# yuan-xy/Audio-Triangulation

Measured on AMD Instinct MI355X. Metric: GCC-PHAT localizations/sec, 3-mic x 1024-sample frames, higher is better.
Workload: dtype f32

## Files before the change

audio-triangulation_amd/csrc/tdoa_capi.cpp:

```cpp

#include "../../include/tdoa.h"
#include "tdoa_devmem.h"
#include "tdoa_internal.h"
#include "tdoa_tables.h"

#include <hip/hip_runtime.h>

#include <cstdlib>

#include <algorithm>
#include <cmath>
#include <cstring>
#include <map>
#include <memory>
#include <mutex>
#include <tuple>
#include <vector>

struct tdoa_ctx {
    tdoa_tables t;
    int device;
    tdoa_devmem window, prior, tuples, tuple_cell, mic, lut;
    tdoa_devmem tw;
    tdoa_devmem p1k_img;
    tdoa_devmem w64_img;
    tdoa_devmem bb;
    tdoa_devmem wc;
    tdoa_devmem fgq;
    tdoa_devmem wscratch;
    tdoa_devmem rscratch, cscratch, tscratch;
    tdoa_devmem pscratch;
    tdoa_devmem spec;
    std::vector<float> bin_w;
    tdoa_devmem d_bin_w;
    tdoa_kparams kp;
};

extern "C" int tdoa_config_default(tdoa_config *cfg)
{
    if (!cfg)
        return tdoa_fail(TDOA_ERR_INVALID, "tdoa_config_default: NULL");
    std::memset(cfg, 0, sizeof *cfg);
    cfg->num_mics = 3;
    cfg->frame_len = 1024;
    cfg->sample_rate_hz = 50000;
    cfg->max_shift = 0;
    cfg->speed_of_sound = 343.0f;
    cfg->engine = TDOA_ENGINE_DIRECT;
    cfg->mic_xy = nullptr;
    cfg->grid_half_w = 50;
    cfg->grid_half_h = 50;
    cfg->grid_scale = 24.0f;
    cfg->height_offset = 1.2f;
    cfg->window_q15 = nullptr;
    cfg->phat_eps = 1e-12f;
    return TDOA_OK;
}

namespace {

int check_device(int device)
{
    int ndev = 0;
    if (hipGetDeviceCount(&ndev) != hipSuccess || ndev <= 0)
        return tdoa_fail(TDOA_ERR_NO_DEVICE, "no HIP device visible (libtdoa has no CPU path)");
    if (device < 0 || device >= ndev)
        return tdoa_fail(TDOA_ERR_INVALID, "device %d out of range (%d visible)", device, ndev);
    hipDeviceProp_t prop;
    HIP_TRY(hipGetDeviceProperties(&prop, device));
    if (std::strncmp(prop.gcnArchName, "gfx950", 6) != 0)
        return tdoa_fail(TDOA_ERR_NO_DEVICE, "device %d is %s; libtdoa is built for gfx950 only",
                         device, prop.gcnArchName);
    return TDOA_OK;
}

template <typename T> size_t vbytes(const std::vector<T> &v) { return v.size() * sizeof(T); }

int upload_tables(tdoa_ctx *c)
{
    const tdoa_tables &t = c->t;
    std::vector<int16_t> w16(t.N);
    for (int i = 0; i < t.N; i++)
        w16[i] = (int16_t)t.win[i];
    if (c->window.alloc(vbytes(w16)) != hipSuccess || c->prior.alloc(vbytes(t.prior)) != hipSuccess ||
        c->tuples.alloc(vbytes(t.tuples)) != hipSuccess || c->tuple_cell.alloc(vbytes(t.tuple_cell)) != hipSuccess ||
        c->mic.alloc(vbytes(t.mic)) != hipSuccess || c->lut.alloc(vbytes(t.lut)) != hipSuccess)
        return tdoa_fail(TDOA_ERR_NOMEM, "hipMalloc of context tables failed");
    hipError_t e = c->window.upload(w16.data(), vbytes(w16));
    if (e == hipSuccess)
        e = c->mic.upload(t.mic.data(), vbytes(t.mic));
    if (e == hipSuccess)
        e = c->lut.upload(t.lut.data(), vbytes(t.lut));
    if (e == hipSuccess)
        e = c->prior.upload(t.prior.data(), vbytes(t.prior));
    if (e == hipSuccess)
        e = c->tuples.upload(t.tuples.data(), vbytes(t.tuples));
    if (e == hipSuccess)
        e = c->tuple_cell.upload(t.tuple_cell.data(), vbytes(t.tuple_cell));
    if (e != hipSuccess)
        return tdoa_fail(TDOA_ERR_HIP, "uploading context tables: %s", hipGetErrorString(e));
    return TDOA_OK;
}

int upload_gcc_phat(tdoa_ctx *c)
{
    const tdoa_tables &t = c->t;
    if (c->tw.upload(t.tw.data(), vbytes(t.tw)) != hipSuccess)
        return tdoa_fail(TDOA_ERR_NOMEM, "uploading twiddle tables failed");
    std::vector<uint8_t> img;
    tdoa_phat1024_image(t.M, t.N, t.K, t.U, t.tw.data(), t.win.data(), t.prior.data(), t.tuples.data(),
                        t.tuple_cell.data(), img);
    if (!img.empty() && c->p1k_img.upload(img.data(), img.size()) != hipSuccess)
        return tdoa_fail(TDOA_ERR_NOMEM, "uploading the GCC_PHAT table image failed");
#if TDOA_AB
    tdoa_p1k_w64_image(t.M, t.N, t.K, t.U, t.win.data(), t.prior.data(), t.tuples.data(), img);
    if (!img.empty() && c->w64_img.upload(img.data(), img.size()) != hipSuccess)
        return tdoa_fail(TDOA_ERR_NOMEM, "uploading the GCC_PHAT (w64) table image failed");
#endif
    if (tdoa_gcc_phat_needs_split(t.M, t.N) && c->spec.alloc(TDOA_SPEC_BYTES) != hipSuccess)
        return tdoa_fail(TDOA_ERR_NOMEM, "GCC_PHAT spectrum scratch of %zu bytes", TDOA_SPEC_BYTES);
    return TDOA_OK;
}

int upload_grid(tdoa_ctx *c)
{
    const tdoa_tables &t = c->t;
    if (t.bb_NT <= 0)
        return TDOA_OK;
    if (c->bb.upload(t.bb_img.data(), t.bb_img.size()) != hipSuccess)
        return tdoa_fail(TDOA_ERR_NOMEM, "uploading the grid tile tables failed");
    if (!t.wc_ok || c->wc.upload(t.wc_chunks.data(), vbytes(t.wc_chunks)) != hipSuccess) {
        c->wc.release();
        return TDOA_OK;
    }
#if TDOA_AB
    if (t.fg_ok && c->fgq.upload(t.fg.data(), vbytes(t.fg)) != hipSuccess)
        c->fgq.release();
#endif
    return TDOA_OK;
}

void wire_kparams(tdoa_ctx *c)
{
    const tdoa_tables &t = c->t;
    tdoa_kparams &kp = c->kp;
    kp = t.kp;
    kp.window = c->window.get<int16_t>();
    kp.prior = c->prior.get<float>();
    kp.mic_xy = c->mic.get<float>();
    kp.lut = c->lut.get<uint8_t>();
    kp.tuples = c->tuples.get<uint32_t>();
    kp.tuple_cell = c->tuple_cell.get<int32_t>();
    kp.tw = c->tw.get<float>();
    kp.tw2 = kp.tw + t.tw2_at;
    kp.r16_tw = kp.tw + t.r16_at;
    kp.p1k_img = c->p1k_img.get<void>();
    kp.p1k_img_bytes = (int32_t)c->p1k_img.bytes();
    kp.w64_img = c->w64_img.get<void>();
    kp.w64_img_bytes = (int32_t)c->w64_img.bytes();
    if (c->bb) {
        const char *b = c->bb.get<char>();
        kp.bb_tile = (const int32_t *)(b + t.bb_at[tdoa_tables::BB_TILE]);
        kp.bb_rng = (const uint16_t *)(b + t.bb_at[tdoa_tables::BB_RNG]);
        kp.bb_tuples = (const uint32_t *)(b + t.bb_at[tdoa_tables::BB_TUPLES]);
        kp.bb_uidx = (const int32_t *)(b + t.bb_at[tdoa_tables::BB_UIDX]);
        kp.bb_q = (const uint16_t *)(b + t.bb_at[tdoa_tables::BB_Q]);
    }
    kp.wc_chunks = c->wc.get<uint32_t>();
    if (!c->wc)
        kp.wc_CK = kp.wc_nch = 0;
#if TDOA_AB
    if (c->fgq) {
        kp.fg_q = c->fgq.get<uint16_t>();
        kp.fg_tup = (const uint16_t *)(c->fgq.get<char>() + t.fg_tup_at);
        kp.fg_ok = 1;
    }
#endif
}

}

extern "C" int tdoa_create(const tdoa_config *cfg, int device, tdoa_ctx **out)
{
    if (!cfg || !out)
        return tdoa_fail(TDOA_ERR_INVALID, "tdoa_create: NULL argument");
    *out = nullptr;
    auto c = std::make_unique<tdoa_ctx>();
    if (const int rc = tdoa_build_tables(cfg, &c->t))
        return rc;
    if (const int rc = check_device(device))
        return rc;
    c->device = device;
    HIP_TRY(hipSetDevice(device));
    if (const int rc = upload_tables(c.get()))
        return rc;
    if (const int rc = upload_gcc_phat(c.get()))
        return rc;
    if (const int rc = upload_grid(c.get()))
        return rc;
    wire_kparams(c.get());
    *out = c.release();
    return TDOA_OK;
}

extern "C" int tdoa_destroy(tdoa_ctx *ctx)
{
    if (!ctx)
        return TDOA_OK;
    (void)hipSetDevice(ctx->device);
    std::unique_ptr<tdoa_ctx> released(ctx);
    return TDOA_OK;
}

extern "C" int tdoa_get_dims(const tdoa_ctx *c, int32_t *M, int32_t *N, int32_t *P,
                             int32_t *K, int32_t *G)
{
    if (!c)
        return tdoa_fail(TDOA_ERR_INVALID, "tdoa_get_dims: NULL ctx");
    if (M)
        *M = c->t.M;
    if (N)
        *N = c->t.N;
    if (P)
        *P = c->t.P;
    if (K)
        *K = c->t.K;
    if (G)
        *G = c->t.G;
    return TDOA_OK;
}

static tdoa_kout to_kout(const tdoa_outputs *o)
{
    tdoa_kout k{};
    k.lags = o->lags;
    k.gate = o->gate;
    k.cell = o->cell;
    k.xy = o->xy;
    k.max_L = o->max_L;
    k.max_Lf = o->max_Lf;
    k.scores = o->scores;
    k.weighted = o->weighted;
    k.scores_f = o->scores_f;
    k.weighted_f = o->weighted_f;
    return k;
}

int tdoa_resident_blocks(const void *kernel, int threads, size_t lds)
{
    static std::mutex mu;
    static std::map<std::tuple<int, const void *, int, size_t>, int> cache;
    int dev = 0;
    (void)hipGetDevice(&dev);
    const auto key = std::make_tuple(dev, kernel, threads, lds);
    std::lock_guard<std::mutex> lk(mu);
    auto it = cache.find(key);
    if (it != cache.end())
        return it->second;
    int per_cu = 0, cus = 0;
    (void)hipDeviceGetAttribute(&cus, hipDeviceAttributeMultiprocessorCount, dev);
    (void)hipOccupancyMaxActiveBlocksPerMultiprocessor(&per_cu, kernel, threads, lds);
    const int r = (per_cu > 0 ? per_cu : 1) * (cus > 0 ? cus : 256);
    cache[key] = r;
    return r;
}

static bool env_flag(const char *name)
{
    const char *e = getenv(name);
    return e && *e && strcmp(e, "0") != 0;
}

static int64_t compact_chunk(int64_t B)
{
    static const int64_t chunk = [] {
        const char *e = getenv("TDOA_F16_CHUNK");
        return e ? (int64_t)atoll(e) : (int64_t)0;
    }();
    return chunk > 0 && chunk < B ? chunk : B;
}

static tdoa_kout offset_kout(const tdoa_kout &k, int64_t c0, int P, int K)
{
    tdoa_kout o = k;
    auto adv = [&](auto *&ptr, int64_t per) {
        if (ptr)
            ptr += c0 * per;
    };
    adv(o.lags, P);
    adv(o.gate, 1);
    adv(o.cell, 1);
    adv(o.xy, 2);
    adv(o.max_L, 1);
    adv(o.max_Lf, 1);
    adv(o.scores, (int64_t)P * K);
    adv(o.weighted, (int64_t)P * K);
    adv(o.scores_f, (int64_t)P * K);
    adv(o.weighted_f, (int64_t)P * K);
    adv(o.peak3, (int64_t)P * 3);
    return o;
}

static int run_compact_chunks(tdoa_ctx *ctx, const tdoa_kout &k, const int16_t *frames, int64_t B, int64_t chunk,
                              const void *weighted, void *stream)
{
    const int64_t M = ctx->kp.M, N = ctx->kp.N;
    int rc = 0;
    for (int64_t c0 = 0; rc == 0 && c0 < B; c0 += chunk) {
        const int64_t n = B - c0 < chunk ? B - c0 : chunk;
        const tdoa_kout kc = offset_kout(k, c0, ctx->t.P, ctx->t.K);
        rc = tdoa_launch_gcc_phat(ctx->kp, kc, frames + c0 * M * N, n, ctx->t.cfg.phat_eps, ctx->spec.get<void>(),
                                  ctx->spec.bytes(), stream);
        if (rc == 0)
            rc = tdoa_launch_grid(ctx->kp, kc, weighted, true, n, stream);
    }
    return rc;
}

static int run_batch(tdoa_ctx *ctx, const int16_t *frames, int64_t B, const tdoa_outputs *out,
                     void *stream, bool prepared)
{
    if (!ctx || !out)
        return tdoa_fail(TDOA_ERR_INVALID, "localize: NULL argument");
    if (B < 0)
        return tdoa_fail(TDOA_ERR_INVALID, "localize: negative batch");
    if (B == 0)
        return TDOA_OK;
    if (!frames)
        return tdoa_fail(TDOA_ERR_INVALID, "localize: NULL frames");
    if (!out->lags)
        return tdoa_fail(TDOA_ERR_INVALID, "localize: outputs.lags is required");
    HIP_TRY(hipSetDevice(ctx->device));
    const bool phat = ctx->t.cfg.engine == TDOA_ENGINE_GCC_PHAT && !prepared;
    tdoa_kout k = to_kout(out);
    const bool ls = out->xy_ls || out->ls_rms;
    const bool grid =
        ls || out->cell || out->xy || (phat ? out->max_Lf != nullptr : out->max_L != nullptr);
    const size_t sz = phat ? sizeof(float) : sizeof(int64_t);
    const size_t pk = (size_t)B * ctx->t.P * ctx->t.K * sz;
    const void *weighted = phat ? (const void *)out->weighted_f : (const void *)out->weighted;
    const bool fused_grid = phat ? tdoa_gcc_phat_grid_in_kernel(ctx->kp) : tdoa_direct_fused_grid(ctx->kp);
    const bool compact = grid && !weighted && !fused_grid && phat && tdoa_gcc_phat_peak3(ctx->kp) &&
                         tdoa_grid_bb_compact(ctx->kp) && !env_flag("TDOA_NO_COMPACT");
    const int64_t chunk = compact ? compact_chunk(B) : B;
    if (compact) {
        if (const int rc = ctx->wscratch.grow((size_t)chunk * ctx->kp.wc_CK * sizeof(float), stream,
                                                    "weighted-score"))
            return rc;
        k.weighted_c = ctx->wscratch.get<float>();
        weighted = k.weighted_c;
    } else if (grid && !weighted && !fused_grid) {
        if (const int rc = ctx->wscratch.grow(pk, stream, "weighted-score"))
            return rc;
        weighted = ctx->wscratch.get<void>();
        if (phat)
            k.weighted_f = ctx->wscratch.get<float>();
        else
            k.weighted = ctx->wscratch.get<int64_t>();
    }
    const void *raw = phat ? (const void *)out->scores_f : (const void *)out->scores;
    const bool peak_k = ls && phat && tdoa_gcc_phat_peak3(ctx->kp);
    if (peak_k) {
        if (const int rc = ctx->tscratch.grow((size_t)B * ctx->t.P * 3 * sizeof(float), stream,
                                                    "peak-score"))
            return rc;
        k.peak3 = ctx->tscratch.get<float>();
    }
    if (ls && !raw && !peak_k) {
        if (const int rc = ctx->rscratch.grow(pk, stream, "raw-score"))
            return rc;
        raw = ctx->rscratch.get<void>();
        if (phat)
            k.scores_f = ctx->rscratch.get<float>();
        else
            k.scores = ctx->rscratch.get<int64_t>();
    }
    if (ls && !out->cell) {
        if (const int rc = ctx->cscratch.grow((size_t)B * 4, stream, "cell"))
            return rc;
        k.cell = ctx->cscratch.get<int32_t>();
    }
    int rc = 0;
    if (compact && chunk < B) {
        rc = run_compact_chunks(ctx, k, frames, B, chunk, weighted, stream);
    } else {
        rc = phat ? tdoa_launch_gcc_phat(ctx->kp, k, frames, B, ctx->t.cfg.phat_eps, ctx->spec.get<void>(),
                                         ctx->spec.bytes(), stream)
                  : tdoa_launch_direct(ctx->kp, k, frames, B, prepared, stream, nullptr);
        if (rc != 0 || !grid)
            return rc;
        if (!fused_grid)
            rc = tdoa_launch_grid(ctx->kp, k, weighted, phat, B, stream);
    }
    if (rc != 0 || !ls)
        return rc;
    return tdoa_launch_ls(ctx->kp, raw, phat, k.peak3, k.lags, k.cell, out->xy_ls, out->ls_rms, B, stream);
}

extern "C" int tdoa_heatmap(tdoa_ctx *ctx, const void *weighted, const void *max_L, int is_float,
                            int64_t B, uint8_t *classes, void *stream)
{
    if (!ctx || !weighted || !max_L || !classes)
        return tdoa_fail(TDOA_ERR_INVALID, "tdoa_heatmap: NULL argument");
    if (B < 0)
        return tdoa_fail(TDOA_ERR_INVALID, "tdoa_heatmap: negative batch");
    HIP_TRY(hipSetDevice(ctx->device));
    return tdoa_launch_heatmap(ctx->kp, weighted, max_L, is_float != 0, B, classes, stream);
}

extern "C" int tdoa_peaks(tdoa_ctx *ctx, const void *scores, int is_float, int64_t B,
                          const tdoa_peaks_params *prm, const tdoa_peaks_outputs *out, void *stream)
{
    if (!ctx || !scores || !prm || !out)
        return tdoa_fail(TDOA_ERR_INVALID, "tdoa_peaks: NULL argument");
    if (!out->cell)
        return tdoa_fail(TDOA_ERR_INVALID, "tdoa_peaks: outputs.cell is required");
    if (B < 0)
        return tdoa_fail(TDOA_ERR_INVALID, "tdoa_peaks: negative batch");
    if (B > INT32_MAX)
        return tdoa_fail(TDOA_ERR_INVALID, "tdoa_peaks: batch too large for one launch");
    if (prm->num_peaks < 1 || prm->num_peaks > TDOA_MAX_PEAKS)
        return tdoa_fail(TDOA_ERR_INVALID, "tdoa_peaks: num_peaks %d outside 1..%d", (int)prm->num_peaks,
                    TDOA_MAX_PEAKS);
    if (prm->radius < 0)
        return tdoa_fail(TDOA_ERR_INVALID, "tdoa_peaks: negative radius");
    if (!tdoa_peaks_fits(ctx->kp, is_float != 0))
        return tdoa_fail(TDOA_ERR_INVALID, "tdoa_peaks: the L map and one frame's scores (%zu bytes) exceed the LDS budget",
                    tdoa_peaks_lds(ctx->kp, is_float != 0));
    if (B == 0)
        return TDOA_OK;
    HIP_TRY(hipSetDevice(ctx->device));
    const int Kp = prm->num_peaks;
    const bool ls = out->xy_ls || out->ls_rms;
    tdoa_peaks_kout k;
    k.count = out->count;
    k.cell = out->cell;
    k.xy = out->xy;
    k.L = out->L;
    k.Lf = out->Lf;
    k.lags = out->lags;
    if (ls && !k.lags) {
        if (const int rc = ctx->pscratch.grow((size_t)B * Kp * ctx->t.P * sizeof(int32_t), stream,
                                                    "peak-lag"))
            return rc;
        k.lags = ctx->pscratch.get<int32_t>();
    }
    int rc = tdoa_launch_peaks(ctx->kp, k, scores, is_float != 0, B, Kp, prm->radius, prm->min_rel, stream);
    if (rc != 0 || !ls)
        return rc;
    return tdoa_launch_ls(ctx->kp, scores, is_float != 0, nullptr, k.lags, k.cell, out->xy_ls, out->ls_rms,
                          B * Kp, stream, Kp);
}

const tdoa_kparams *tdoa_ctx_kparams(const tdoa_ctx *c) { return &c->kp; }
int tdoa_ctx_device(const tdoa_ctx *c) { return c->device; }
int tdoa_ctx_engine(const tdoa_ctx *c) { return c->t.cfg.engine; }
int tdoa_ctx_rate(const tdoa_ctx *c) { return c->t.cfg.sample_rate_hz; }

extern "C" int tdoa_localize_batch(tdoa_ctx *ctx, const int16_t *frames, int64_t B,
                                   const tdoa_outputs *out, void *stream)
{
    return run_batch(ctx, frames, B, out, stream, false);
}

extern "C" int tdoa_correlate_prepared(tdoa_ctx *ctx, const int16_t *prepared, int64_t B,
                                       const tdoa_outputs *out, void *stream)
{
    return run_batch(ctx, prepared, B, out, stream, true);
}

extern "C" int tdoa_average_batch(tdoa_ctx *ctx, int64_t S, int64_t *est, const int64_t *fresh,
                                  const float *decay, int32_t *best, const tdoa_outputs *solve,
                                  void *stream)
{
    if (!ctx || !est || !fresh || !decay || !best)
        return tdoa_fail(TDOA_ERR_INVALID, "tdoa_average_batch: NULL argument");
    if (S < 0)
        return tdoa_fail(TDOA_ERR_INVALID, "tdoa_average_batch: negative stream count");
    if (S == 0)
        return TDOA_OK;
    HIP_TRY(hipSetDevice(ctx->device));
    tdoa_kout k;
    const tdoa_kout *kptr = nullptr;
    if (solve) {
        k = to_kout(solve);
        kptr = &k;
    }
    return tdoa_launch_average(ctx->kp, S, est, fresh, decay, best, kptr, stream);
}

extern "C" float tdoa_decay_us(uint64_t now_us, uint64_t last_us)
{
    const float dt = (float)(now_us - last_us) / 1e6f;
    const float arg = -dt / 0.5f;
    return (float)(1.0 - std::exp((double)arg));
}

extern "C" int tdoa_get_window(const tdoa_ctx *c, int32_t *w)
{
    if (!c || !w)
        return tdoa_fail(TDOA_ERR_INVALID, "NULL");
    std::memcpy(w, c->t.win.data(), sizeof(int32_t) * c->t.N);
    return TDOA_OK;
}

extern "C" int tdoa_get_mics(const tdoa_ctx *c, float *xy)
{
    if (!c || !xy)
        return tdoa_fail(TDOA_ERR_INVALID, "NULL");
    std::memcpy(xy, c->t.mic.data(), sizeof(float) * 2 * c->t.M);
    return TDOA_OK;
}

extern "C" int tdoa_get_lut(const tdoa_ctx *c, uint8_t *lut)
{
    if (!c || !lut)
        return tdoa_fail(TDOA_ERR_INVALID, "NULL");
    std::memcpy(lut, c->t.lut.data(), c->t.lut.size());
    return TDOA_OK;
}

extern "C" int tdoa_get_prior(const tdoa_ctx *c, float *scale)
{
    if (!c || !scale)
        return tdoa_fail(TDOA_ERR_INVALID, "NULL");
    std::memcpy(scale, c->t.prior.data(), sizeof(float) * c->t.K);
    return TDOA_OK;
}

extern "C" int tdoa_set_bin_weights(tdoa_ctx *ctx, const float *w)
{
    if (!ctx)
        return tdoa_fail(TDOA_ERR_INVALID, "tdoa_set_bin_weights: NULL ctx");
    if (ctx->t.cfg.engine != TDOA_ENGINE_GCC_PHAT)
        return tdoa_fail(TDOA_ERR_INVALID, "tdoa_set_bin_weights: the context's engine is not GCC_PHAT");
    if (!w) {
        ctx->bin_w.clear();
        ctx->kp.bin_w = nullptr;
        ctx->kp.bin_lo = ctx->kp.bin_hi = 0;
        return TDOA_OK;
    }
    const int n = ctx->t.N + 1;
    int lo = -1, hi = -1;
    for (int k = 0; k < n; k++) {
        if (!std::isfinite(w[k]) || w[k] < 0.0f)
            return tdoa_fail(TDOA_ERR_INVALID, "tdoa_set_bin_weights: w[%d] is negative or not finite", k);
        if (w[k] != 0.0f) {
            lo = lo < 0 ? k : lo;
            hi = k;
        }
    }
    if (lo < 0)
        return tdoa_fail(TDOA_ERR_INVALID, "tdoa_set_bin_weights: every weight is zero");
    HIP_TRY(hipSetDevice(ctx->device));
    if (!ctx->spec && ctx->spec.alloc(TDOA_SPEC_BYTES) != hipSuccess)
        return tdoa_fail(TDOA_ERR_NOMEM, "GCC_PHAT spectrum scratch of %zu bytes", TDOA_SPEC_BYTES);
    if (!ctx->d_bin_w && ctx->d_bin_w.alloc(sizeof(float) * n) != hipSuccess)
        return tdoa_fail(TDOA_ERR_NOMEM, "tdoa_set_bin_weights: weight table of %d floats", n);
    HIP_TRY(ctx->d_bin_w.upload(w, sizeof(float) * n));
    ctx->bin_w.assign(w, w + n);
    ctx->kp.bin_w = ctx->d_bin_w.get<float>();
    ctx->kp.bin_lo = lo;
    ctx->kp.bin_hi = hi;
    return TDOA_OK;
}

extern "C" int tdoa_set_band_hz(tdoa_ctx *ctx, double lo_hz, double hi_hz, double taper_hz)
{
    if (!ctx)
        return tdoa_fail(TDOA_ERR_INVALID, "tdoa_set_band_hz: NULL ctx");
    std::vector<float> w((size_t)ctx->t.N + 1);
    const int rc = tdoa_band_weights(ctx->t.N, ctx->t.cfg.sample_rate_hz, lo_hz, hi_hz, taper_hz, w.data());
    return rc ? rc : tdoa_set_bin_weights(ctx, w.data());
}

extern "C" int tdoa_get_bin_weights(const tdoa_ctx *c, float *w)
{
    if (!c || !w)
        return tdoa_fail(TDOA_ERR_INVALID, "NULL");
    if (c->bin_w.empty())
        std::fill(w, w + c->t.N + 1, 1.0f);
    else
        std::memcpy(w, c->bin_w.data(), sizeof(float) * c->bin_w.size());
    return TDOA_OK;
}


extern "C" const char *tdoa_batch_kernel(const tdoa_ctx *ctx)
{
    if (!ctx)
        return "";
    if (ctx->t.cfg.engine == TDOA_ENGINE_GCC_PHAT)
        return tdoa_gcc_phat_kernel_name(ctx->kp);
    return tdoa_direct_fused_grid(ctx->kp) ? "k_direct_mfma" : "k_direct";
}

extern "C" int tdoa_batch_grid_fused(const tdoa_ctx *ctx)
{
    if (!ctx)
        return 0;
    return (ctx->t.cfg.engine == TDOA_ENGINE_GCC_PHAT ? tdoa_gcc_phat_grid_in_kernel(ctx->kp)
                                                    : tdoa_direct_fused_grid(ctx->kp))
               ? 1
               : 0;
}

extern "C" int tdoa_abi_version(void) { return TDOA_ABI_VERSION; }
```

audio-triangulation_amd/csrc/tdoa_internal.h:

```cpp
#pragma once

#include <stddef.h>
#include <stdint.h>

#include <vector>

#include <hip/hip_runtime.h>

#include "tdoa_shared.h"

__device__ __forceinline__ void wave_lds_sync()
{
    __builtin_amdgcn_fence(__ATOMIC_RELEASE, "wavefront");
    __builtin_amdgcn_wave_barrier();
    __builtin_amdgcn_fence(__ATOMIC_ACQUIRE, "wavefront");
}

__device__ __forceinline__ double ls_tau3(double y0, double y1, double y2, int best, bool inside)
{
#pragma clang fp contract(off)
    double d = 0.0;
    if (inside) {
        const double den = y0 - 2.0 * y1 + y2;
        if (den < 0.0) {
            d = 0.5 * (y0 - y2) / den;
            d = d < -0.5 ? -0.5 : (d > 0.5 ? 0.5 : d);
        }
    }
    return (double)best + d;
}

__device__ __forceinline__ float tdoa_decay_dev(uint64_t now, uint64_t last)
{
#pragma clang fp contract(off)
    const float dt = (float)(now - last) / 1e6f;
    const float arg = -dt / 0.5f;
    return (float)(1.0 - exp((double)arg));
}

struct tdoa_kout {
    int32_t *lags;
    uint8_t *gate;
    int32_t *cell;
    float *xy;
    int64_t *max_L;
    float *max_Lf;
    int64_t *scores;
    int64_t *weighted;
    float *scores_f;
    float *weighted_f;
    float *peak3;
    float *weighted_c;
};

struct tdoa_peaks_kout {
    int32_t *count;
    int32_t *cell;
    float *xy;
    int64_t *L;
    float *Lf;
    int32_t *lags;
};

struct tdoa_stream_params {
    int32_t M, N, H, log2N, fs;
    int64_t capture_len;
    const uint8_t *capture;
    int64_t *pos;
    int64_t *ring_start;
    int32_t *count;
    int32_t *count_next;
    int32_t *ids;
    int64_t *end;
    int64_t *ring_at;
    int16_t *frames;
    int64_t *fresh;
    int32_t *fresh_lags;
    uint8_t *fresh_gate;
    int64_t *est;
    uint64_t *last;
    int64_t *stats;
};

struct tdoa_stream_kout {
    int32_t *count;
    int32_t *stream_id;
    int64_t *end;
    int32_t *lags;
    uint8_t *gate;
    int32_t *ema_best;
    int32_t *cell;
    float *xy;
    int64_t *max_L;
};

int tdoa_resident_blocks(const void *kernel, int threads, size_t lds);

struct tdoa_stream_fuse {
    tdoa_stream_params sp;
    tdoa_stream_kout so;
};
int tdoa_launch_direct(const tdoa_kparams &kp, const tdoa_kout &out,
                       const int16_t *frames, int64_t B, bool prepared,
                       void *stream, int *lds_bytes_out,
                       const int32_t *count_dev = nullptr, const tdoa_stream_fuse *ema = nullptr);
bool tdoa_direct_fused_grid(const tdoa_kparams &kp);
bool tdoa_direct_ema_fits(const tdoa_kparams &kp);
int tdoa_launch_heatmap(const tdoa_kparams &kp, const void *weighted, const void *max_L,
                        bool is_float, int64_t B, uint8_t *classes, void *stream);
int tdoa_launch_ls(const tdoa_kparams &kp, const void *scores, bool is_float, const float *peak3,
                   const int32_t *lags, const int32_t *cells, float *xy_ls, float *rms,
                   int64_t B, void *stream, int per_frame = 0);
size_t tdoa_peaks_lds(const tdoa_kparams &kp, bool is_float);
bool tdoa_peaks_fits(const tdoa_kparams &kp, bool is_float);
int tdoa_launch_peaks(const tdoa_kparams &kp, const tdoa_peaks_kout &out, const void *scores,
                      bool is_float, int64_t B, int num_peaks, int radius, float min_rel,
                      void *stream);
size_t tdoa_stream_trigger_lds(int M, int N, int H);
int tdoa_launch_stream_trigger(const tdoa_stream_params &sp, int64_t S, void *stream, bool *by_id);
int tdoa_launch_stream_update(const tdoa_stream_params &sp, const tdoa_kparams &kp,
                              const tdoa_stream_kout &out, int64_t S, void *stream);
int tdoa_launch_average(const tdoa_kparams &kp, int64_t S, int64_t *est,
                        const int64_t *fresh, const float *decay, int32_t *best,
                        const tdoa_kout *solve, void *stream);
int tdoa_launch_grid(const tdoa_kparams &kp, const tdoa_kout &out, const void *weighted,
                     bool is_float, int64_t B, void *stream);
int tdoa_launch_gcc_phat(const tdoa_kparams &kp, const tdoa_kout &out,
                         const int16_t *frames, int64_t B, float phat_eps,
                         void *spec_scratch, size_t spec_bytes, void *stream);
bool tdoa_gcc_phat_needs_split(int M, int N);
void tdoa_phat1024_image(int M, int N, int K, int U, const float *tw, const int32_t *win,
                         const float *prior, const uint32_t *tuples, const int32_t *tuple_cell,
                         std::vector<uint8_t> &img);
void tdoa_p1k_w64_image(int M, int N, int K, int U, const int32_t *win, const float *prior,
                        const uint32_t *tuples, std::vector<uint8_t> &img);
bool tdoa_gcc_phat_fused_grid(const tdoa_kparams &kp);
bool tdoa_phat1024_fits(const tdoa_kparams &kp);
int tdoa_launch_phat1024(const tdoa_kparams &kp, const tdoa_kout &out, const int16_t *frames,
                         int64_t B, float phat_eps, void *stream);
bool tdoa_p1k_w64_fits(const tdoa_kparams &kp);
int tdoa_launch_p1k_w64(const tdoa_kparams &kp, const tdoa_kout &out, const int16_t *frames, int64_t B,
                        float phat_eps, void *stream);
bool tdoa_phat_r16_fits(int M, int N, int S);
bool frame16_shape(const tdoa_kparams &kp);
const char *frame16_kernel_name(const tdoa_kparams &kp);
bool tdoa_phat_r16_peak3(const tdoa_kparams &kp);
bool tdoa_frame16_fused_grid(const tdoa_kparams &kp);
int tdoa_launch_phat_r16(const tdoa_kparams &kp, const tdoa_kout &out, const int16_t *frames, int64_t B,
                         float phat_eps, void *scratch, size_t scratch_bytes, void *stream);
const char *tdoa_gcc_phat_kernel_name(const tdoa_kparams &kp);
bool tdoa_grid_bb_compact(const tdoa_kparams &kp);
bool tdoa_gcc_phat_grid_in_kernel(const tdoa_kparams &kp);
bool tdoa_gcc_phat_peak3(const tdoa_kparams &kp);
int tdoa_launch_gcc_phat_split(const tdoa_kparams &kp, const tdoa_kout &out,
                               const int16_t *frames, int64_t B, float eps_int16,
                               void *scratch, size_t scratch_bytes, void *stream);
int tdoa_launch_ref_buffer(int op, int16_t *buf, const int16_t *ring, int head, int64_t *power,
                           const int16_t *window, int n, void *stream, int16_t *s1, int16_t *s2);

struct tdoa_ctx;
const tdoa_kparams *tdoa_ctx_kparams(const tdoa_ctx *c);
int tdoa_ctx_device(const tdoa_ctx *c);
int tdoa_ctx_engine(const tdoa_ctx *c);
int tdoa_ctx_rate(const tdoa_ctx *c);
```

audio-triangulation_amd/csrc/tdoa_phat1024.hip:

```cpp
#include <hip/hip_runtime.h>
#include <stdint.h>

#include <algorithm>
#include <climits>
#include <cstdio>
#include <cstdlib>
#include <map>
#include <type_traits>
#include <vector>

#include "tdoa_cplx.h"
#include "tdoa_internal.h"


namespace {

constexpr int P1K_ROW = 264;
constexpr int P1K_TILE = 32 * P1K_ROW;
constexpr int P1K_KPAD = 128;
constexpr int P1K_WAVE_LDS = 2 * P1K_TILE;
[[maybe_unused]] constexpr int P1K_GB = 8;
constexpr int P1K_IMG_FIXED = 32 * 32 * 8 + 16 * 32 * 8 + 512 * 8 + 128 * 4;

__host__ __device__ constexpr int slot(int x) { return x == 16 ? 24 : (x == 24 ? 16 : x); }

__device__ __forceinline__ int lane_res(int l)
{
    return l < 2 ? l * 16 : ((l & 1) ? 32 - (l >> 1) : (l >> 1));
}

__device__ __forceinline__ float dpp_xor1(float v)
{
    return __builtin_bit_cast(
        float, __builtin_amdgcn_mov_dpp(__builtin_bit_cast(int, v), 0xB1, 0xF, 0xF, false));
}
__device__ __forceinline__ f2 dpp_xor1(f2 v) { return f2{dpp_xor1(v.x), dpp_xor1(v.y)}; }
typedef short v2s_t __attribute__((ext_vector_type(2)));

#define P1K_X(i) "%" #i
#define P1K_DPP(i) "v_mov_b32_dpp " P1K_X(i) ", " P1K_X(i) " quad_perm:[1,0,3,2] row_mask:0xf bank_mask:0xf\n\t"
#define P1K_MOV(d, s) "v_mov_b64 " P1K_X(d) ", " P1K_X(s) "\n\t"
template <bool FWD, int NV>
__device__ __forceinline__ void swap_upper_exec(f2 (&V)[NV], f2 E)
{
    float x[32];
#pragma unroll
    for (int j = 0; j < 16; j++) {
        x[2 * j] = V[16 + j].x;
        x[2 * j + 1] = V[16 + j].y;
    }
    uint64_t sv;
    asm volatile("s_mov_b64 %[sv], exec\n\t"
                 "s_and_b64 exec, exec, %[m1]\n\t"
                 "s_nop 4\n\t" P1K_DPP(0) P1K_DPP(1) P1K_DPP(2) P1K_DPP(3) P1K_DPP(4) P1K_DPP(5)
                     P1K_DPP(6) P1K_DPP(7) P1K_DPP(8) P1K_DPP(9) P1K_DPP(10) P1K_DPP(11) P1K_DPP(12)
                         P1K_DPP(13) P1K_DPP(14) P1K_DPP(15) P1K_DPP(16) P1K_DPP(17) P1K_DPP(18)
                             P1K_DPP(19) P1K_DPP(20) P1K_DPP(21) P1K_DPP(22) P1K_DPP(23) P1K_DPP(24)
                                 P1K_DPP(25) P1K_DPP(26) P1K_DPP(27) P1K_DPP(28) P1K_DPP(29)
                                     P1K_DPP(30) P1K_DPP(31) "s_mov_b64 exec, %[sv]\n\t"
                 "s_nop 4"
                 : "+v"(x[0]), "+v"(x[1]), "+v"(x[2]), "+v"(x[3]), "+v"(x[4]), "+v"(x[5]),
                   "+v"(x[6]), "+v"(x[7]), "+v"(x[8]), "+v"(x[9]), "+v"(x[10]), "+v"(x[11]),
                   "+v"(x[12]), "+v"(x[13]), "+v"(x[14]), "+v"(x[15]), "+v"(x[16]), "+v"(x[17]),
                   "+v"(x[18]), "+v"(x[19]), "+v"(x[20]), "+v"(x[21]), "+v"(x[22]), "+v"(x[23]),
                   "+v"(x[24]), "+v"(x[25]), "+v"(x[26]), "+v"(x[27]), "+v"(x[28]), "+v"(x[29]),
                   "+v"(x[30]), "+v"(x[31]), [sv] "=&s"(sv)
                 : [m1] "s"(0xFFFFFFFCFFFFFFFCull));
    f2 y[16];
#pragma unroll
    for (int j = 0; j < 16; j++)
        y[j] = f2{x[2 * j], x[2 * j + 1]};
    const f2 e = FWD ? V[0] : E;
#define P1K_ROT_ASM(ROT)                                                                            \
    asm volatile("s_mov_b64 %[sv], exec\n\t"                                                        \
                 "s_and_b64 exec, exec, %[m2]\n\t"                                                  \
                 "s_nop 4\n\t" ROT "s_mov_b64 exec, %[sv]\n\t"                                     \
                 "s_nop 4"                                                                           \
                 : "+v"(y[0]), "+v"(y[1]), "+v"(y[2]), "+v"(y[3]), "+v"(y[4]), "+v"(y[5]),           \
                   "+v"(y[6]), "+v"(y[7]), "+v"(y[8]), "+v"(y[9]), "+v"(y[10]), "+v"(y[11]),         \
                   "+v"(y[12]), "+v"(y[13]), "+v"(y[14]), "+v"(y[15]), [sv] "=&s"(sv)                \
                 : [m2] "s"(0x0000000100000001ull), [e] "v"(e))
    if constexpr (FWD)
        P1K_ROT_ASM(P1K_MOV(0, 1) P1K_MOV(1, 2) P1K_MOV(2, 3) P1K_MOV(3, 4) P1K_MOV(4, 5) P1K_MOV(5, 6)
                        P1K_MOV(6, 7) P1K_MOV(7, 8) P1K_MOV(8, 9) P1K_MOV(9, 10) P1K_MOV(10, 11)
                            P1K_MOV(11, 12) P1K_MOV(12, 13) P1K_MOV(13, 14) P1K_MOV(14, 15)
                                "v_mov_b64 %15, %[e]\n\t");
    else
        P1K_ROT_ASM(P1K_MOV(15, 14) P1K_MOV(14, 13) P1K_MOV(13, 12) P1K_MOV(12, 11) P1K_MOV(11, 10)
                        P1K_MOV(10, 9) P1K_MOV(9, 8) P1K_MOV(8, 7) P1K_MOV(7, 6) P1K_MOV(6, 5)
                            P1K_MOV(5, 4) P1K_MOV(4, 3) P1K_MOV(3, 2) P1K_MOV(2, 1) P1K_MOV(1, 0)
                                "v_mov_b64 %0, %[e]\n\t");
#undef P1K_ROT_ASM
#pragma unroll
    for (int j = 0; j < 16; j++)
        V[16 + j] = y[j];
}

__device__ __forceinline__ int hsum32(int s, int hw)
{
    s += __builtin_amdgcn_mov_dpp(s, 0xB1, 0xF, 0xF, false);
    s += __builtin_amdgcn_mov_dpp(s, 0x4E, 0xF, 0xF, false);
    s += __builtin_amdgcn_mov_dpp(s, 0x141, 0xF, 0xF, false);
    s += __builtin_amdgcn_mov_dpp(s, 0x140, 0xF, 0xF, false);
    s += __builtin_amdgcn_update_dpp(0, s, 0x142, 0xA, 0xF, false);
    const int s0 = __builtin_amdgcn_readlane(s, 31), s1 = __builtin_amdgcn_readlane(s, 63);
    return hw ? s1 : s0;
}

#ifndef P1K_VLDS
#define P1K_VLDS 1
#endif
__device__ __forceinline__ f2 lds_f2(const char *base, int off)
{
#if P1K_VLDS
    return lds_rd(reinterpret_cast<const f2 *>(base + off));
#else
    return *reinterpret_cast<const f2 *>(base + off);
#endif
}
#ifndef P1K_GROUPS
#define P1K_GROUPS 0
#endif
#ifndef P1K_CELL_LDS
#define P1K_CELL_LDS 0
#endif
#ifndef P1K_BALANCE
#define P1K_BALANCE 1
#endif
#ifndef P1K_W2_EARLY
#define P1K_W2_EARLY 0
#endif
#ifndef P1K_LATE_STORES
#define P1K_LATE_STORES 1
#endif
__device__ __forceinline__ f2 lds_f2_plain(const char *base, int off)
{
    return *reinterpret_cast<const f2 *>(base + off);
}
__device__ __forceinline__ f2 lds_at(uint32_t addr)
{
    return *(const __attribute__((address_space(3))) f2 *)(uintptr_t)addr;
}
__device__ __forceinline__ void sts_f2(char *base, int off, f2 v)
{
    *reinterpret_cast<f2 *>(base + off) = v;
}

__device__ __forceinline__ void pin(f2 &x) { asm volatile("" : "+v"(x)); }


struct Lane {
    int hw;
    int lane;
    int res;
    int cs;
    bool is0, is1;
    char *tileA;
    const char *twm;
    const char *tw2;
    const char *win;
};

template <bool INV, bool HALF_ZERO>
__device__ __forceinline__ void fft_col_lds(const Lane &L, f2 (&v)[32], char *tile)
{
    fft32d<INV, HALF_ZERO>(v);
    wave_lds_sync();
    const int wo = 8 * L.cs;
#pragma unroll
    for (int k0 = 0; k0 < 32; k0 += 8) {
        f2 tw[8];
#pragma unroll
        for (int i = 0; i < 8; i++)
            tw[i] = lds_f2(L.twm, wo + 256 * (k0 + i));
#pragma unroll
        for (int i = 0; i < 8; i++) {
            const int k = k0 + i;
            f2 x = v[k];
            if (k)
                x = INV ? c_mulconj(x, tw[i]) : c_mul(x, tw[i]);
            sts_f2(tile, wo + P1K_ROW * slot(k), x);
        }
    }
    wave_lds_sync();
}
__device__ __forceinline__ void fft_row_fwd(const Lane &L, const char *tile, f2 (&V)[33])
{
    f2 v[32];
    const int ro = P1K_ROW * L.cs;
#pragma unroll
    for (int n = 0; n < 32; n++)
        v[n] = lds_f2(tile, ro + 8 * slot(n));
    fft32d<false, false>(v);
#pragma unroll
    for (int k = 0; k < 32; k++)
        V[k] = v[k];
}
}

#ifdef TDOA_DIAG
__device__ unsigned long long g_diag_p1k[1 << 16];
#endif

namespace {

struct NoHook {
    __device__ void operator()() const {}
};

template <typename Hook = NoHook>
__device__ __forceinline__ void lean_spectrum(const Lane &L, const uint32_t (&w)[16], f2 (&V)[33],
                                              float e2, Hook after_front = Hook())
{
    f2 v[32];
    {
        int s = 0;
#pragma unroll
        for (int t = 0; t < 16; t++)
            s = __builtin_amdgcn_sdot2(__builtin_bit_cast(v2s_t, w[t]), v2s_t{1, 1}, s, false);
        s = hsum32(s, L.hw);
        const uint32_t off = (uint32_t)(s >> 10) & 0xFFu;
        const uint32_t off2 = off | (off << 16);
#pragma unroll
        for (int t = 0; t < 16; t++) {
            const f2 wf = lds_f2(L.win, 8 * L.cs + 256 * t);
            const uint32_t d = (w[t] | 0x01000100u) - off2;
            const float s0 = (float)(int8_t)(d & 0xFFu);
            const float s1 = (float)(int8_t)((d >> 16) & 0xFFu);
            const f2 pr = f2{s0, s1} * wf;
            v[t] = f2{floorf(pr.x), floorf(pr.y)};
        }
    }
    after_front();
    fft_col_lds<false, true>(L, v, L.tileA);
    float e2q;
    asm volatile("v_ldexp_f32 %0, %1, -2" : "=v"(e2q) : "s"(e2));
    fft_row_fwd(L, L.tileA, V);
    V[32] = c_unit(conjf2(V[16]), e2q);
    swap_upper_exec<true>(V, f2{0.0f, 0.0f});
}

__device__ __forceinline__ void lean_split_w(f2 A, f2 Bv, f2 wk, float e2, f2 &ub, f2 &un)
{
    const f2 e = c_addconj(A, Bv);
    const f2 od = c_mul(c_subconj(A, Bv), wk);
    ub = c_unit(c_add_mi(e, od), e2);
    un = c_unit(c_conj_add_i(e, od), e2);
}
#ifndef P1K_TWPF
#define P1K_TWPF 5
#endif
__device__ __forceinline__ f2 lean_tw2(const Lane &L, int k) { return lds_f2(L.tw2, 8 * L.cs + 256 * k); }
__device__ __forceinline__ void lean_split(const Lane &L, f2 A, f2 Bv, int k, float e2, f2 &ub,
                                           f2 &un)
{
    lean_split_w(A, Bv, lean_tw2(L, k), e2, ub, un);
}

template <typename Hook = NoHook>
__device__ __forceinline__ void lean_forward(const Lane &L, const uint32_t (&w)[16], f2 (&U)[33],
                                             float e2, Hook after_front = Hook())
{
    lean_spectrum(L, w, U, e2, after_front);
#if P1K_TWPF & 1
    f2 wn = lean_tw2(L, 0);
#pragma unroll
    for (int k = 0; k < 16; k++) {
        const f2 wk = wn;
        if (k < 15)
            wn = lean_tw2(L, k + 1);
        lean_split_w(U[k], U[31 - k], wk, e2, U[k], U[31 - k]);
    }
#else
#pragma unroll
    for (int k = 0; k < 16; k++)
        lean_split(L, U[k], U[31 - k], k, e2, U[k], U[31 - k]);
#endif
}

__device__ __forceinline__ void lean_forward_cross(const Lane &L, const uint32_t (&w)[16],
                                                   f2 (&A)[33], f2 (&Bs)[33], float e2)
{
    f2 V[33];
    lean_spectrum(L, w, V, e2);
    A[32] = c_conjmul(A[32], V[32]);
    Bs[32] = c_conjmul(Bs[32], V[32]);
#if P1K_TWPF & 2
    f2 wn = lean_tw2(L, 0);
#endif
#pragma unroll
    for (int k = 0; k < 16; k++) {
        f2 ub, un;
#if P1K_TWPF & 2
        const f2 wk = wn;
        if (k < 15)
            wn = lean_tw2(L, k + 1);
        lean_split_w(V[k], V[31 - k], wk, e2, ub, un);
#else
        lean_split(L, V[k], V[31 - k], k, e2, ub, un);
#endif
        A[k] = c_conjmul(A[k], ub);
        A[31 - k] = c_conjmul(A[31 - k], un);
        Bs[k] = c_conjmul(Bs[k], ub);
        Bs[31 - k] = c_conjmul(Bs[31 - k], un);
    }
}

__device__ __forceinline__ f2 cmac_fwd(f2 acc, f2 d, int k)
{
    if (k == 0)
        return acc + d;
    if (k == 8)
        return c_add_mi(acc, d);
    const f2 w = f2{(float)COS32D[k], -(float)COS32D[k < 8 ? 8 - k : k - 8]};
    return v_fma(v_yy(d), f2{-w.y, w.x}, v_fma(v_xx(d), w, acc));
}

__device__ __forceinline__ void lean_row_inv(const Lane &L, const char *tile, f2 &y0, f2 &y31)
{
    const int ro = P1K_ROW * L.cs;
    f2 ga[2], gd[2];
#pragma unroll
    for (int g = 0; g < 2; g++) {
        f2 a[8], c[2];
#pragma unroll
        for (int i = 0; i < 8; i++) {
            const f2 v = lds_f2(tile, ro + 8 * slot(8 * g + i));
            const f2 u = lds_f2(tile, ro + 8 * slot(8 * g + i + 16));
            a[i] = v + u;
            const f2 d = v - u;
            c[i & 1] = i < 2 ? tw_only<false>(d, 8 * g + i) : cmac_fwd(c[i & 1], d, 8 * g + i);
        }
#pragma unroll
        for (int h = 4; h >= 1; h >>= 1)
#pragma unroll
            for (int r = 0; r < h; r++)
                a[r] = a[r] + a[r + h];
        ga[g] = a[0];
        gd[g] = c[0] + c[1];
        pin(ga[g]);
        pin(gd[g]);
    }
    y0 = ga[0] + ga[1];
    y31 = gd[0] + gd[1];
}

__device__ __forceinline__ int lane_res_sel(int l)
{
    const int h = l >> 1, o = l & 1;
    return h + o * (32 - 2 * h) - ((l == 1) << 4);
}


__device__ __forceinline__ int fresh_tid()
{
    int t = (int)threadIdx.x;
    asm volatile("" : "+v"(t));
    return t;
}

template <bool CROSS>
__device__ __forceinline__ void lean_pretwiddle(const Lane &L, const f2 (&A)[33], const f2 (&Bs)[33],
                                                f2 (&v)[32])
{
#if P1K_TWPF & 4
    f2 wn = lean_tw2(L, 0);
#endif
#pragma unroll
    for (int k = 0; k < 16; k++) {
        const f2 Rk = CROSS ? c_conjmul(A[k], Bs[k]) : A[k];
        const f2 Rn = CROSS ? c_conjmul(A[31 - k], Bs[31 - k]) : A[31 - k];
#if P1K_TWPF & 4
        const f2 wk = wn;
        if (k < 15)
            wn = lean_tw2(L, k + 1);
#else
        const f2 wk = lean_tw2(L, k);
#endif
        const f2 s = c_addconj(Rk, Rn);
        const f2 q = c_mulconj(c_subconj(Rk, Rn), wk);
        v[k] = c_add_i(s, q);
        v[31 - k] = c_conj_add_mi(s, q);
    }
    const f2 R32 = CROSS ? c_conjmul(A[32], Bs[32]) : A[32];
    const f2 Ye = f2{2.0f * R32.x, -2.0f * R32.y};
    swap_upper_exec<false>(v, Ye);
}

}

__global__ void __launch_bounds__(512, 2) k_p1k_lean(tdoa_kparams kp, tdoa_kout out,
                                                     const int16_t *__restrict__ frames, int64_t B,
                                                     float e2)
{
    constexpr int N = 1024, P = 3, NW = 8, NF = 2 * NW, NT = NW * 64;
    extern __shared__ __attribute__((aligned(16))) char smem[];
    char *tiles = smem;
    char *twm = tiles + NW * 2 * P1K_TILE;
    char *tw2 = twm + 32 * 32 * 8;
    char *win = tw2 + 16 * 32 * 8;
    const float *prior = (const float *)(win + 512 * 8);
    const uint32_t *tups = (const uint32_t *)(prior + 128);

    const int tid = threadIdx.x, wave = tid >> 6, hw = (tid >> 5) & 1, lane64 = tid & 63;
#ifdef TDOA_DIAG
    unsigned long long stamp[16] = {};
    int nst = 0;
#define LEAN_MARK()                                               \
    do {                                                          \
        if (nst < 16)                                             \
            stamp[nst++] = __builtin_amdgcn_s_memtime();          \
    } while (0)
    stamp[nst++] = __builtin_amdgcn_s_memtime();
    stamp[14] = __builtin_amdgcn_s_memrealtime();
#else
#define LEAN_MARK() \
    do {            \
    } while (0)
#endif
    __shared__ int prog[NW];
    if (lane64 == 0)
        prog[wave] = 0;
    __builtin_amdgcn_s_setprio(2);
    int phase = 0;
    auto balance = [&]() {
#if P1K_BALANCE
        volatile __attribute__((address_space(3))) int *pv = (volatile __attribute__((address_space(3))) int *)prog;
        ++phase;
        if (lane64 == 0)
            pv[wave] = phase;
        const int other = __builtin_amdgcn_readfirstlane(pv[wave ^ 4]);
        if (phase > other)
            __builtin_amdgcn_s_setprio(0);
        else
            __builtin_amdgcn_s_setprio(2);
#endif
    };
    Lane L;
    L.hw = hw;
    L.lane = tid & 31;
    L.res = lane_res(L.lane);
    L.cs = slot(L.res);
    L.is0 = L.lane == 0;
    L.is1 = L.lane == 1;
    char *wtiles = tiles + wave * 2 * P1K_TILE;
    L.tileA = wtiles + hw * P1K_TILE;
    L.twm = twm;
    L.tw2 = tw2;
    L.win = win;

    const int K = kp.K, S = kp.S;
    const bool do_grid = out.cell || out.xy || out.max_Lf;
#if !P1K_GROUPS
    const int Upad = (kp.U + P1K_GB * 64 - 1) / (P1K_GB * 64) * (P1K_GB * 64);
#endif

    auto fetch = [&](uint32_t(&w)[16], int64_t fr, int m) {
        const uint32_t *row = reinterpret_cast<const uint32_t *>(
            frames + ((fr < B ? fr : B - 1) * 3 + m) * (int64_t)N) + L.res;
#pragma unroll
        for (int t = 0; t < 16; t++)
            w[t] = __builtin_nontemporal_load(row + 32 * t);
    };
    uint32_t w0[16], w1[16];
    {
        const uint4 *src = (const uint4 *)kp.p1k_img;
        uint4 *dst = (uint4 *)twm;
        const int n16 = do_grid ? kp.p1k_img_bytes / 16 : P1K_IMG_FIXED / 16;
        constexpr int SR = 4;
        uint4 img[SR];
#pragma unroll
        for (int r = 0; r < SR; r++)
            img[r] = src[tid + r * NT < n16 ? tid + r * NT : n16 - 1];
        const int64_t f = (int64_t)blockIdx.x * NF + 2 * wave + hw;
        fetch(w0, f, 0);
#pragma unroll
        for (int r = 0; r < SR; r++)
            dst[tid + r * NT < n16 ? tid + r * NT : n16 - 1] = img[r];
    }
    __syncthreads();
#pragma unroll
    for (int t = 0; t < 16; t++)
        asm volatile("" : "+v"(w0[t]));

    const float invL = 1.0f / 2048.0f;

    {
        const int64_t base = (int64_t)blockIdx.x * NF;
        const int64_t f = base + 2 * wave + hw;
        const bool live = f < B;
        uint32_t w2[16];
        LEAN_MARK();
        float wv[3][4];
        int best[3];
        auto finish_pair = [&](int p, f2 y0, f2 y31) {
            const int ft = fresh_tid();
            const int fres = lane_res_sel(ft & 31), fhw = (ft >> 5) & 1;
            const int la = 2 * fres, lb = 2 * fres - 64;
            const int ck[4] = {lb + S, lb + 1 + S, la + S, la + 1 + S};
            const bool ok[4] = {lb >= -S, lb + 1 >= -S, la <= S, la + 1 <= S};
            const float cv[4] = {y31.x * invL, y31.y * invL, y0.x * invL, y0.y * invL};
            int bkey = INT_MIN, bk = INT_MAX;
#pragma unroll
            for (int c = 0; c < 4; c++) {
                const int kc = fkey(cv[c]);
                if (ok[c] && kc > bkey) {
                    bkey = kc;
                    bk = ck[c];
                }
            }
            half_argmax_key(bkey, bk);
            bk = bk < 0 ? 0 : (bk >= K ? K - 1 : bk);
            best[p] = bk - S;
            const int64_t ff = base + 2 * ((ft >> 6) & 7) + fhw;
#pragma unroll
            for (int c = 0; c < 4; c++) {
                const int d = ck[c] > bk ? ck[c] - bk : bk - ck[c];
                wv[p][c] = ok[c] ? cv[c] * prior[ok[c] ? d : 0] : 0.0f;
            }
            if (out.scores_f || out.weighted_f) {
                float *sr = out.scores_f ? out.scores_f + (size_t)(ff * P + p) * K : nullptr;
                float *wr = out.weighted_f ? out.weighted_f + (size_t)(ff * P + p) * K : nullptr;
#pragma unroll
                for (int c = 0; c < 4; c++)
                    if (ff < B && ok[c]) {
                        if (sr)
                            sr[ck[c]] = cv[c];
                        if (wr)
                            wr[ck[c]] = wv[p][c];
                    }
            }
#if !P1K_LATE_STORES
            if (ff < B && (ft & 31) == 0)
                out.lags[ff * P + p] = bk - S;
#endif
        };

        f2 U0[33], U1[33], y0, y31;
        lean_forward(L, w0, U0, e2, [&] {
            fetch(w1, f, 1);
            balance();
        });
        LEAN_MARK();
        balance();
#if P1K_W2_EARLY
        lean_forward(L, w1, U1, e2, [&] {
            fetch(w2, f, 2);
            balance();
        });
#else
        lean_forward(L, w1, U1, e2, [&] { balance(); });
#endif
        LEAN_MARK();
        balance();
        {
            f2 v[32];
            lean_pretwiddle<true>(L, U0, U1, v);
            fft_col_lds<true, false>(L, v, L.tileA);
#if !P1K_W2_EARLY
            fetch(w2, f, 2);
#endif
            lean_row_inv(L, L.tileA, y0, y31);
        }
        finish_pair(0, y0, y31);
        LEAN_MARK();
        balance();
        lean_forward_cross(L, w2, U0, U1, e2);
        LEAN_MARK();
        balance();
        {
            f2 v[32];
            lean_pretwiddle<false>(L, U0, U0, v);
            fft_col_lds<true, false>(L, v, L.tileA);
            lean_row_inv(L, L.tileA, y0, y31);
        }
        finish_pair(1, y0, y31);
        LEAN_MARK();
        balance();
        {
            f2 v[32];
            lean_pretwiddle<false>(L, U1, U1, v);
            fft_col_lds<true, false>(L, v, L.tileA);
            lean_row_inv(L, L.tileA, y0, y31);
        }
        finish_pair(2, y0, y31);
        LEAN_MARK();
        balance();
        auto store_frame = [&]() {
            if (live && L.lane == 0) {
#pragma unroll
                for (int p = 0; p < 3; p++)
                    out.lags[f * P + p] = best[p];
                if (out.gate)
                    out.gate[f] = best[0] * best[0] + best[1] * best[1] + best[2] * best[2] > 4 ? 1 : 0;
            }
        };
#if !P1K_LATE_STORES
        store_frame();
#endif
        if (!do_grid) {
#if P1K_LATE_STORES
            store_frame();
#endif
            return;
        }
        wave_lds_sync();
#if P1K_CELL_LDS && !P1K_GROUPS
        float *wsc = (float *)(((uintptr_t)wtiles + 1023) & ~(uintptr_t)1023);
#else
        float *wsc = (float *)wtiles;
#endif
        const int gres = lane_res_sel(fresh_tid() & 31);
        const int gla = 2 * gres, glb = 2 * gres - 64;
        const int ck[4] = {glb + S, glb + 1 + S, gla + S, gla + 1 + S};
        const bool ok[4] = {glb >= -S, glb + 1 >= -S, gla <= S, gla + 1 <= S};
#pragma unroll
        for (int p = 0; p < P; p++)
#pragma unroll
            for (int c = 0; c < 4; c++)
                if (ok[c])
                    wsc[(p * P1K_KPAD + ck[c]) * 2 + hw] = wv[p][c];
        {
            const int ft = fresh_tid();
            if ((ft & 31) < 3)
                wsc[((ft & 31) * P1K_KPAD + P1K_KPAD - 1) * 2 + ((ft >> 5) & 1)] = -INFINITY;
        }
        wave_lds_sync();
        LEAN_MARK();
#if P1K_GROUPS
        const int *ghdr = reinterpret_cast<const int *>(static_cast<const char *>(kp.p1k_img) + P1K_IMG_FIXED);
        const int gn3 = ghdr[0], gn2 = ghdr[1], gn1 = ghdr[2], gcell0 = ghdr[3];
        const uint32_t *gw = tups + 4;
        const uint16_t *gcl = reinterpret_cast<const uint16_t *>(gw + gn3 + gn2 + gn1);
        const int gcb2 = 3 * gn3, gcb1 = gcb2 + 2 * gn2, gend = gn3 + gn2 + gn1;
        float gv[2] = {-INFINITY, -INFINITY};
        int gs[2] = {0, 0}, gsl[2] = {0, 0};
        const char *ws = (const char *)wsc;
        constexpr int R1 = P1K_KPAD * 8, R2 = 2 * P1K_KPAD * 8;
        auto gat = [&](auto nm, uint32_t w, f2 &a, f2 &b, f2 (&c)[decltype(nm)::value]) {
            a = lds_rd(reinterpret_cast<const f2 *>(ws + (w & 0x3FFu)));
            b = lds_rd(reinterpret_cast<const f2 *>(ws + R1 + ((w >> 10) & 0x3FFu)));
#pragma unroll
            for (int j = 0; j < decltype(nm)::value; j++)
                c[j] = lds_rd(reinterpret_cast<const f2 *>(ws + R2 + (w >> 20) + 8 * j));
        };
        auto bucket = [&](auto nm, int s0, int s1) {
            constexpr int NM = decltype(nm)::value;
            if (s0 >= s1)
                return;
            const int last = s1 - 64;
            const int nu = (s1 - s0) / 128;
            auto words = [&](uint32_t (&w)[2], int u) {
                w[0] = lds_rd_u32(gw + imin(s0 + 128 * u, last) + lane64);
                w[1] = lds_rd_u32(gw + imin(s0 + 128 * u + 64, last) + lane64);
            };
            auto gather = [&](const uint32_t (&w)[2], f2 (&a)[2], f2 (&b)[2], f2 (&c)[2][NM]) {
                gat(nm, w[0], a[0], b[0], c[0]);
                gat(nm, w[1], a[1], b[1], c[1]);
            };
            auto consume = [&](const f2 (&a)[2], const f2 (&b)[2], const f2 (&c)[2][NM], int u) {
#pragma unroll
                for (int r = 0; r < 2; r++) {
                    const f2 part = a[r] + b[r];
                    f2 L[NM];
#pragma unroll
                    for (int j = 0; j < NM; j++)
                        L[j] = part + c[r][j];
                    float m[2] = {L[0].x, L[0].y};
#pragma unroll
                    for (int j = 1; j < NM; j++) {
                        m[0] = fmaxf(m[0], L[j].x);
                        m[1] = fmaxf(m[1], L[j].y);
                    }
                    const int sl = s0 + 128 * u + 64 * r + lane64;
#pragma unroll
                    for (int f = 0; f < 2; f++) {
                        const bool gt = m[f] > gv[f];
                        gsl[f] = m[f] >= gv[f] ? sl : gsl[f];
                        gs[f] = gt ? sl : gs[f];
                        gv[f] = gt ? m[f] : gv[f];
                    }
                }
            };
            f2 a0[2], b0[2], c0[2][NM], a1[2], b1[2], c1[2][NM];
            uint32_t w2[2], w3[2];
            words(w2, 0);
            gather(w2, a0, b0, c0);
            words(w3, 1);
            words(w2, 2);
            gather(w3, a1, b1, c1);
            int u = 0;
            for (; u + 3 < nu; u += 2) {
                consume(a0, b0, c0, u);
                words(w3, u + 3);
                gather(w2, a0, b0, c0);
                __builtin_amdgcn_sched_barrier(0);
                consume(a1, b1, c1, u + 1);
                words(w2, u + 4);
                gather(w3, a1, b1, c1);
                __builtin_amdgcn_sched_barrier(0);
            }
            consume(a0, b0, c0, u);
            if (u + 2 < nu)
                gather(w2, a0, b0, c0);
            if (u + 1 < nu)
                consume(a1, b1, c1, u + 1);
            if (u + 2 < nu)
                consume(a0, b0, c0, u + 2);
        };
        bucket(std::integral_constant<int, 3>{}, 0, gn3);
        bucket(std::integral_constant<int, 2>{}, gn3, gn3 + gn2);
        bucket(std::integral_constant<int, 1>{}, gn3 + gn2, gend);
        LEAN_MARK();
        auto group_cell = [&](int sl, int f, float v) {
            const int nm = sl < gn3 ? 3 : (sl < gn3 + gn2 ? 2 : 1);
            const int cb = sl < gn3 ? 3 * sl : (sl < gn3 + gn2 ? gcb2 + 2 * (sl - gn3) : gcb1 + (sl - gn3 - gn2));
            const uint32_t w = gw[sl];
            const f2 part = lds_f2_plain(ws, (int)(w & 0x3FFu)) + lds_f2_plain(ws, R1 + (int)((w >> 10) & 0x3FFu));
            int mc = INT_MAX;
#pragma unroll
            for (int j = 0; j < 3; j++) {
                if (j < nm) {
                    const f2 Lg = part + lds_f2_plain(ws, R2 + (int)(w >> 20) + 8 * j);
                    if ((f ? Lg.y : Lg.x) == v)
                        mc = imin(mc, (int)gcl[cb + j]);
                }
            }
            return mc;
        };
        int cand[2];
        {
            uint32_t bw[2];
            int bnm[2], bc[2][3];
#pragma unroll
            for (int f = 0; f < 2; f++) {
                const int sl = gs[f];
                bnm[f] = sl < gn3 ? 3 : (sl < gn3 + gn2 ? 2 : 1);
                const int cb = sl < gn3 ? 3 * sl : (sl < gn3 + gn2 ? gcb2 + 2 * (sl - gn3) : gcb1 + (sl - gn3 - gn2));
                bw[f] = gw[sl];
#pragma unroll
                for (int j = 0; j < 3; j++)
                    bc[f][j] = gcl[cb + imin(j, bnm[f] - 1)];
            }
#pragma unroll
            for (int f = 0; f < 2; f++) {
                const uint32_t w = bw[f];
                const f2 part = lds_f2_plain(ws, (int)(w & 0x3FFu)) + lds_f2_plain(ws, R1 + (int)((w >> 10) & 0x3FFu));
                int mc = INT_MAX;
#pragma unroll
                for (int j = 0; j < 3; j++) {
                    const f2 Lg = part + lds_f2_plain(ws, R2 + (int)(w >> 20) + 8 * j);
                    if (j < bnm[f] && (f ? Lg.y : Lg.x) == gv[f])
                        mc = imin(mc, bc[f][j]);
                }
                cand[f] = gv[f] > -INFINITY ? mc : INT_MAX;
            }
        }
        int wcell[2];
#pragma unroll
        for (int j = 0; j < 2; j++) {
            int ci = cand[j];
            int gk = fkey(gv[j]);
            wave_argmax_key(gk, ci);
            const float V = fkey_value(gk);
            if (__ballot(gsl[j] != gs[j] && gv[j] == V && V > -INFINITY)) {
                int mc = INT_MAX;
                for (int sl = lane64; sl < gend; sl += 64)
                    mc = imin(mc, group_cell(sl, j, V));
                ci = wave_reduce<false>(mc);
            }
            wcell[j] = ci == INT_MAX ? gcell0 : ci;
            gv[j] = V;
        }
        LEAN_MARK();
#else
        float gv[2] = {-INFINITY, -INFINITY};
        int gu[2] = {INT_MAX, INT_MAX};
        const char *ws = (const char *)wsc;
#if P1K_CELL_LDS
        const uint32_t wsb = (uint32_t)(uintptr_t)(const __attribute__((address_space(3))) char *)ws;
#endif
        auto gather = [&](const uint32_t (&qq)[4], f2 (&g)[4][3]) {
#pragma unroll
            for (int i = 0; i < 4; i++) {
#if P1K_CELL_LDS
                g[i][0] = lds_at((qq[i] & 0x3F8u) | wsb);
                g[i][1] = lds_at((((qq[i] >> 7) & 0x3F8u) | wsb) + P1K_KPAD * 8);
                g[i][2] = lds_at((((qq[i] >> 14) & 0x3F8u) | wsb) + 2 * P1K_KPAD * 8);
#else
                g[i][0] = lds_f2_plain(ws, (int)(qq[i] & 0x3FFu));
                g[i][1] = lds_f2_plain(ws, P1K_KPAD * 8 + (int)((qq[i] >> 10) & 0x3FFu));
                g[i][2] = lds_f2_plain(ws, 2 * P1K_KPAD * 8 + (int)(qq[i] >> 20));
#endif
            }
        };
        uint32_t q[4];
        f2 g[4][3];
#pragma unroll
        for (int i = 0; i < 4; i++)
            q[i] = tups[64 * i + lane64];
        gather(q, g);
        auto consume = [&](const f2 (&gg)[4][3], int ub) {
#pragma unroll
            for (int i = 0; i < 4; i++) {
                const f2 Lg = (gg[i][0] + gg[i][1]) + gg[i][2];
                const int u = ub + 64 * i + lane64;
                if (Lg.x > gv[0]) {
                    gv[0] = Lg.x;
                    gu[0] = u;
                }
                if (Lg.y > gv[1]) {
                    gv[1] = Lg.y;
                    gu[1] = u;
                }
            }
        };
        for (int u0 = 0; u0 < Upad; u0 += 512) {
            uint32_t qn[4];
#pragma unroll
            for (int i = 0; i < 4; i++)
                qn[i] = tups[u0 + 256 + 64 * i + lane64];
            f2 gn[4][3];
            gather(qn, gn);
            consume(g, u0);
            const int un = u0 + 512 < Upad ? u0 + 512 : u0 + 256;
#pragma unroll
            for (int i = 0; i < 4; i++)
                q[i] = tups[un + 64 * i + lane64];
            gather(q, g);
            consume(gn, u0 + 256);
        }
        LEAN_MARK();
        int mycell[2], myu[2];
#if P1K_CELL_LDS
        const int *rowcell = reinterpret_cast<const int *>(tups + Upad);
#pragma unroll
        for (int j = 0; j < 2; j++) {
            myu[j] = gu[j];
            const int uc = (gu[j] < 0 || gu[j] >= kp.U) ? 0 : gu[j];
            const uint32_t tw = tups[uc];
            mycell[j] = rowcell[uc >> 5] + (int)((tw >> 24) | ((tw & 7u) << 8));
        }
#else
#pragma unroll
        for (int j = 0; j < 2; j++) {
            myu[j] = gu[j];
            mycell[j] = kp.tuple_cell[(gu[j] < 0 || gu[j] >= kp.U) ? 0 : gu[j]];
        }
#endif
        int gk[2];
#pragma unroll
        for (int j = 0; j < 2; j++) {
            gk[j] = fkey(gv[j]);
            wave_argmax_key(gk[j], gu[j]);
            gv[j] = fkey_value(gk[j]);
        }
        LEAN_MARK();
        int wcell[2];
#if P1K_CELL_LDS
        const int tuple_cell0 = rowcell[0];
#else
        const int tuple_cell0 = kp.tuple_cell[0];
#endif
#pragma unroll
        for (int j = 0; j < 2; j++) {
            const int fu = gu[j];
            const uint64_t wm = __ballot(myu[j] == fu && fu >= 0 && fu < kp.U);
            wcell[j] = wm ? __builtin_amdgcn_readlane(mycell[j], __builtin_ctzll(wm)) : tuple_cell0;
        }
#endif
        if (lane64 == 63) {
            const int cells[2] = {wcell[0], wcell[1]};
#pragma unroll
            for (int j = 0; j < 2; j++) {
                const int64_t fs = base + 2 * wave + j;
                if (fs < B) {
                    if (out.cell)
                        out.cell[fs] = cells[j];
                    if (out.max_Lf)
                        out.max_Lf[fs] = gv[j];
                    if (out.xy) {
                        const int cx = cells[j] % kp.grid_W, cy = cells[j] / kp.grid_W;
                        out.xy[2 * fs] = (float)(cx - kp.half_w) / kp.grid_scale;
                        out.xy[2 * fs + 1] = (float)(kp.half_h - cy) / kp.grid_scale;
                    }
                }
            }
        }
#if P1K_LATE_STORES
        store_frame();
#endif
        LEAN_MARK();
    }
#ifdef TDOA_DIAG
    stamp[13] = __builtin_amdgcn_s_memtime();
    stamp[15] = __builtin_amdgcn_s_memrealtime();
    if (lane64 == 0 && (blockIdx.x * NW + wave) < 4096)
        for (int i = 0; i < 16; i++)
            g_diag_p1k[(blockIdx.x * NW + wave) * 16 + i] = stamp[i];
#endif
#undef LEAN_MARK
}

#ifdef TDOA_DIAG
extern "C" int tdoa_diag_fetch_p1k(unsigned long long *host, int n)
{
    if (n > (1 << 16))
        n = 1 << 16;
    return hipMemcpyFromSymbol(host, HIP_SYMBOL(g_diag_p1k), sizeof(unsigned long long) * n, 0,
                               hipMemcpyDeviceToHost) == hipSuccess
               ? 0
               : -2;
}
#endif

namespace {
constexpr int P1K_NW = 8;

constexpr size_t p1k_lds(int img_bytes) { return (size_t)P1K_NW * P1K_WAVE_LDS + (size_t)img_bytes; }
}

void tdoa_phat1024_image(int M, int N, int K, int U, const float *tw, const int32_t *win,
                         const float *prior, const uint32_t *tuples, const int32_t *tuple_cell,
                         std::vector<uint8_t> &img)
{
    img.clear();
    if (M != 3 || N != 1024 || K > P1K_KPAD - 1)
        return;
#if P1K_GROUPS
    struct Grp {
        int l0, l1, l2, n, u0;
        int cell[3];
    };
    std::map<std::pair<int, int>, std::vector<std::pair<int, int>>> by;
    for (int u = 0; u < U; u++)
        by[{(int)(tuples[u] & 0xFFu), (int)((tuples[u] >> 8) & 0xFFu)}].push_back({(int)((tuples[u] >> 16) & 0xFFu), u});
    std::vector<Grp> bk[4];
    for (auto &kv : by) {
        auto &v = kv.second;
        std::sort(v.begin(), v.end());
        for (size_t i = 0; i < v.size();) {
            Grp g{kv.first.first, kv.first.second, v[i].first, 0, INT_MAX, {0, 0, 0}};
            while (i < v.size() && g.n < 3 && v[i].first == g.l2 + g.n) {
                if (tuple_cell[v[i].second] < 0 || tuple_cell[v[i].second] >= 0xFFFF)
                    return;
                g.cell[g.n++] = tuple_cell[v[i].second];
                g.u0 = std::min(g.u0, v[i].second);
                i++;
            }
            bk[g.n].push_back(g);
        }
    }
    int nslot[4];
    for (int n = 1; n <= 3; n++) {
        std::sort(bk[n].begin(), bk[n].end(), [](const Grp &x, const Grp &y) { return x.u0 < y.u0; });
        nslot[n] = ((int)bk[n].size() + 127) / 128 * 128;
    }
    const int ncell = 3 * nslot[3] + 2 * nslot[2] + nslot[1];
    const size_t bytes = (size_t)P1K_IMG_FIXED + 16 + 4 * (size_t)(nslot[3] + nslot[2] + nslot[1]) + 2 * (size_t)ncell;
    img.resize((bytes + 15) / 16 * 16);
#else
    const int Upad = (U + P1K_GB * 64 - 1) / (P1K_GB * 64) * (P1K_GB * 64);
#if P1K_CELL_LDS
    img.resize((size_t)P1K_IMG_FIXED + (size_t)Upad * 4 + (size_t)(Upad / 32) * 4);
#else
    (void)tuple_cell;
    img.resize((size_t)P1K_IMG_FIXED + (size_t)Upad * 4);
#endif
#endif
    float *f = (float *)img.data();
    const float *tw2 = tw + 2 * N;
    for (int k = 0; k < 32; k++)
        for (int r = 0; r < 32; r++) {
            const int i = (k * r) & (N - 1);
            f[2 * (32 * k + slot(r))] = tw[2 * i];
            f[2 * (32 * k + slot(r)) + 1] = tw[2 * i + 1];
        }
    f += 2 * 1024;
    for (int k = 0; k < 16; k++)
        for (int r = 0; r < 32; r++) {
            const int b = r + 32 * k;
            f[2 * (32 * k + slot(r))] = tw2[2 * b];
            f[2 * (32 * k + slot(r)) + 1] = tw2[2 * b + 1];
        }
    f += 2 * 512;
    for (int e = 0; e < 512; e++) {
        const int d = (e & ~31) + slot(e & 31);
        f[2 * d] = (float)win[2 * e] * (1.0f / 128.0f);
        f[2 * d + 1] = (float)win[2 * e + 1] * (1.0f / 128.0f);
    }
    f += 2 * 512;
    for (int k = 0; k < 128; k++)
        f[k] = k < K ? prior[k] : 0.0f;
    uint32_t *t = (uint32_t *)(f + 128);
#if P1K_GROUPS
    int32_t *hdr = (int32_t *)t;
    hdr[0] = nslot[3];
    hdr[1] = nslot[2];
    hdr[2] = nslot[1];
    hdr[3] = U > 0 ? tuple_cell[0] : 0;
    t += 4;
    uint16_t *cl = (uint16_t *)(t + nslot[3] + nslot[2] + nslot[1]);
    for (int n = 3; n >= 1; n--) {
        for (int e = 0; e < nslot[n]; e++) {
            const bool real = e < (int)bk[n].size();
            const Grp g = real ? bk[n][e] : Grp{127, 127, 128 - n, n, 0, {0xFFFF, 0xFFFF, 0xFFFF}};
            *t++ = ((uint32_t)g.l0 << 3) | ((uint32_t)g.l1 << 13) | ((uint32_t)g.l2 << 23);
            for (int j = 0; j < n; j++)
                *cl++ = (uint16_t)g.cell[j];
        }
    }
#else
#if P1K_CELL_LDS
    int32_t *rowcell = (int32_t *)(t + Upad);
    for (int r = 0; r < Upad / 32; r++) {
        const int e0 = 32 * r, e1 = std::min(U, e0 + 32) - 1;
        rowcell[r] = e0 >= U ? 0 : tuple_cell[e0];
        if (e0 < U && tuple_cell[e1] - tuple_cell[e0] >= 2048) {
            img.clear();
            return;
        }
    }
    for (int e = 0; e < Upad; e++) {
        const uint32_t wd = e < U ? tuples[e] : 0x007F7F7Fu;
        const uint32_t dc = e < U ? (uint32_t)(tuple_cell[e] - rowcell[e >> 5]) : 0u;
        t[e] = ((wd & 0x7Fu) << 3) | (((wd >> 8) & 0x7Fu) << 10) | (((wd >> 16) & 0x7Fu) << 17) |
               ((dc & 0xFFu) << 24) | (dc >> 8);
    }
#else
    for (int e = 0; e < Upad; e++) {
        const uint32_t wd = e < U ? tuples[e] : 0x007F7F7Fu;
        t[e] = ((wd & 0xFFu) << 3) | (((wd >> 8) & 0xFFu) << 13) | (((wd >> 16) & 0xFFu) << 23);
    }
#endif
#endif
}

bool tdoa_phat1024_fits(const tdoa_kparams &kp)
{
    if (kp.M != 3 || kp.N != 1024 || kp.S > 63 || kp.TW != 1 || !kp.p1k_img)
        return false;
    static_assert(3 * P1K_KPAD * 8 <= P1K_WAVE_LDS, "grid scores exceed the wave's tiles");
    return kp.p1k_img_bytes <= 4 * P1K_NW * 64 * 16 && p1k_lds(kp.p1k_img_bytes) + 64 <= 160 * 1024;
}

int tdoa_launch_phat1024(const tdoa_kparams &kp, const tdoa_kout &out, const int16_t *frames,
                         int64_t B, float phat_eps, void *stream)
{
    float e2 = phat_eps * 4294967296.0f;
    if (!(e2 >= 1e-30f))
        e2 = 1e-30f;
    if (B <= 0)
        return 0;
    constexpr int NF = 2 * P1K_NW;
    const int64_t grid = (B + NF - 1) / NF;
    if (grid > 0x7FFFFFFF)
        return tdoa_set_error(-1, "k_p1k_lean: batch too large for one launch");
    hipLaunchKernelGGL(k_p1k_lean, dim3((unsigned)grid), dim3(P1K_NW * 64), p1k_lds(kp.p1k_img_bytes), (hipStream_t)stream,
                       kp, out, frames, B, e2);
    const hipError_t e = hipGetLastError();
    if (e != hipSuccess) {
        char buf[256];
        snprintf(buf, sizeof buf, "k_p1k_lean launch: %s", hipGetErrorString(e));
        return tdoa_set_error(-2, buf);
    }
    return 0;
}
```

audio-triangulation_amd/csrc/tdoa_tables.cpp:

```cpp

#include "tdoa_tables.h"

#include "tdoa_bb_layout.h"

#include <algorithm>
#include <cmath>
#include <cstdarg>
#include <cstdio>
#include <cstring>
#include <map>
#include <string>
#include <vector>

namespace {

thread_local std::string g_err;

}

int tdoa_set_error(int code, const char *msg)
{
    g_err = msg;
    return code;
}

int tdoa_fail(int code, const char *fmt, ...)
{
    char buf[512];
    va_list ap;
    va_start(ap, fmt);
    vsnprintf(buf, sizeof buf, fmt, ap);
    va_end(ap);
    return tdoa_set_error(code, buf);
}

extern "C" const char *tdoa_last_error(void) { return g_err.c_str(); }

namespace {

int ilog2(int n)
{
    int b = 0;
    while ((1 << b) < n)
        b++;
    return b;
}

int sturm_count_below(const std::vector<double> &d, const std::vector<double> &e2, double x)
{
    int cnt = 0;
    double q = d[0] - x;
    if (q < 0)
        cnt++;
    for (size_t i = 1; i < d.size(); i++) {
        if (q == 0.0)
            q = 1e-300;
        q = d[i] - x - e2[i] / q;
        if (q < 0)
            cnt++;
    }
    return cnt;
}

void tridiag_solve_pivoted(const std::vector<double> &d, const std::vector<double> &e,
                           double lam, std::vector<double> &b)
{
    const int n = (int)d.size();
    std::vector<double> a(n), c(n), u2(n, 0.0), l(n, 0.0), dd(n);
    std::vector<int> piv(n, 0);
    for (int i = 0; i < n; i++) {
        dd[i] = d[i] - lam;
        a[i] = i > 0 ? e[i] : 0.0;
        c[i] = i + 1 < n ? e[i + 1] : 0.0;
    }
    for (int i = 0; i < n - 1; i++) {
        if (std::fabs(dd[i]) >= std::fabs(a[i + 1])) {
            double f = dd[i] != 0.0 ? a[i + 1] / dd[i] : 0.0;
            if (dd[i] == 0.0)
                dd[i] = 1e-300;
            l[i] = f;
            dd[i + 1] -= f * c[i];
            b[i + 1] -= f * b[i];
            u2[i] = 0.0;
            piv[i] = 0;
        } else {
            double f = dd[i] / a[i + 1];
            l[i] = f;
            double t_d = a[i + 1], t_c = dd[i + 1], t_u2 = i + 2 < n ? c[i + 1] : 0.0;
            double nd1 = c[i] - f * t_c;
            double nu2 = -f * t_u2;
            dd[i] = t_d;
            c[i] = t_c;
            u2[i] = t_u2;
            dd[i + 1] = nd1;
            if (i + 2 < n)
                c[i + 1] = nu2;
            double tb = b[i];
            b[i] = b[i + 1];
            b[i + 1] = tb - f * b[i];
            piv[i] = 1;
        }
    }
    if (dd[n - 1] == 0.0)
        dd[n - 1] = 1e-300;
    b[n - 1] /= dd[n - 1];
    if (n > 1)
        b[n - 2] = (b[n - 2] - c[n - 2] * b[n - 1]) / dd[n - 2];
    for (int i = n - 3; i >= 0; i--)
        b[i] = (b[i] - c[i] * b[i + 1] - u2[i] * b[i + 2]) / dd[i];
}

}

extern "C" int tdoa_dpss_q15(int32_t n, double nw, int32_t *out)
{
    if (n < 4 || !out || !(nw > 0))
        return tdoa_fail(TDOA_ERR_INVALID, "tdoa_dpss_q15: bad arguments");
    const double W = nw / n, cw = std::cos(2.0 * M_PI * W);
    std::vector<double> d(n), e(n, 0.0), e2(n, 0.0);
    for (int i = 0; i < n; i++) {
        const double t = (n - 1 - 2.0 * i) / 2.0;
        d[i] = t * t * cw;
    }
    for (int i = 1; i < n; i++) {
        e[i] = i * (double)(n - i) / 2.0;
        e2[i] = e[i] * e[i];
    }
    double lo = 1e300, hi = -1e300;
    for (int i = 0; i < n; i++) {
        double r = std::fabs(e[i]) + (i + 1 < n ? std::fabs(e[i + 1]) : 0.0);
        lo = std::min(lo, d[i] - r);
        hi = std::max(hi, d[i] + r);
    }
    for (int it = 0; it < 200; it++) {
        double mid = 0.5 * (lo + hi);
        if (mid <= lo || mid >= hi)
            break;
        if (sturm_count_below(d, e2, mid) >= n)
            hi = mid;
        else
            lo = mid;
    }
    const double lam = 0.5 * (lo + hi);
    std::vector<double> v(n, 1.0);
    for (int it = 0; it < 4; it++) {
        tridiag_solve_pivoted(d, e, lam, v);
        double nrm = 0;
        for (double x : v)
            nrm += x * x;
        nrm = std::sqrt(nrm);
        for (double &x : v)
            x /= nrm;
    }
    double s = 0, mx = 0;
    for (double x : v)
        s += x;
    if (s < 0)
        for (double &x : v)
            x = -x;
    for (double x : v)
        mx = std::max(mx, std::fabs(x));
    for (int i = 0; i < n; i++)
        out[i] = (int32_t)std::nearbyint(v[i] / mx * 32767.0);
    return TDOA_OK;
}

extern "C" int tdoa_band_weights(int32_t N, int32_t fs, double lo_hz, double hi_hz, double taper_hz,
                                 float *w)
{
    if (!w)
        return tdoa_fail(TDOA_ERR_INVALID, "tdoa_band_weights: NULL table");
    if (N < 256 || N > 4096 || (N & (N - 1)))
        return tdoa_fail(TDOA_ERR_INVALID, "tdoa_band_weights: N %d must be a power of two in [256,4096]", (int)N);
    if (fs <= 0 || !(lo_hz >= 0.0) || !(lo_hz < hi_hz) || !(hi_hz <= 0.5 * fs) || !(taper_hz >= 0.0) ||
        !std::isfinite(taper_hz))
        return tdoa_fail(TDOA_ERR_INVALID, "tdoa_band_weights: need 0 <= lo < hi <= fs/2 and a finite taper >= 0");
    std::vector<float> t((size_t)N + 1);
    bool any = false;
    for (int k = 0; k <= N; k++) {
        const double f = (double)k * (double)fs / (2.0 * N);
        double v = 0.0;
        if (f >= lo_hz && f <= hi_hz)
            v = 1.0;
        else if (taper_hz > 0.0 && f > lo_hz - taper_hz && f < lo_hz)
            v = 0.5 * (1.0 - std::cos(M_PI * (f - (lo_hz - taper_hz)) / taper_hz));
        else if (taper_hz > 0.0 && f > hi_hz && f < hi_hz + taper_hz)
            v = 0.5 * (1.0 + std::cos(M_PI * (f - hi_hz) / taper_hz));
        t[k] = (float)v;
        any |= t[k] != 0.0f;
    }
    if (!any)
        return tdoa_fail(TDOA_ERR_INVALID, "tdoa_band_weights: no bin of the band has a non-zero weight");
    std::memcpy(w, t.data(), sizeof(float) * t.size());
    return TDOA_OK;
}

namespace {

void reference_triangle(float *xy)
{
    const float dAB = 0.132f, dBC = 0.15f, dCA = 0.20f;
    const float xC = (dAB * dAB + dCA * dCA - dBC * dBC) / (2.0f * dAB);
    const float yC = sqrtf(fmaxf(0.0f, dCA * dCA - xC * xC));
    const float pAx = 0.0f, pAy = 0.0f, pBx = dAB, pBy = 0.0f;
    const float pCx = xC, pCy = yC * -1.0f;
    const float cx = (pAx + pBx + pCx) / 3.0f;
    const float cy = (pAy + pBy + pCy) / 3.0f;
    xy[0] = pAx - cx;
    xy[1] = pAy - cy;
    xy[2] = pBx - cx;
    xy[3] = pBy - cy;
    xy[4] = pCx - cx;
    xy[5] = pCy - cy;
}

inline float hypot3(float x, float y, float z) { return sqrtf(x * x + y * y + z * z); }

void build_lut(tdoa_tables *c)
{
    const int W = c->W, H = c->H, G = c->G;
    const float scale = c->cfg.grid_scale, hgt = c->cfg.height_offset;
    const float sos = c->cfg.speed_of_sound;
    const int fs = c->cfg.sample_rate_hz;
    c->lut.assign((size_t)c->P * G, 0);
    std::vector<float> d(c->M);
    for (int y = 0; y < H; y++)
        for (int x = 0; x < W; x++) {
            float xm = (float)(x - c->cfg.grid_half_w) / scale;
            float ym = (float)(c->cfg.grid_half_h - y) / scale;
            float zm = hgt;
            const float k = hgt / hypot3(zm, xm, ym);
            xm *= k;
            ym *= k;
            zm *= k;
            for (int m = 0; m < c->M; m++)
                d[m] = hypot3(zm, xm - c->mic[2 * m], ym - c->mic[2 * m + 1]);
            int p = 0;
            for (int i = 0; i < c->M; i++)
                for (int j = i + 1; j < c->M; j++, p++) {
                    const float dt = (d[j] - d[i]) / sos;
                    int s = (int)roundf(dt * (float)fs);
                    s = std::min(std::max(s, -c->S), c->S);
                    c->lut[(size_t)p * G + (size_t)y * W + x] = (uint8_t)(s + c->S);
                }
        }
    std::map<std::vector<uint8_t>, int> seen;
    c->tuples.clear();
    c->tuple_cell.clear();
    std::vector<uint8_t> key(c->P);
    for (int cell = 0; cell < G; cell++) {
        for (int p = 0; p < c->P; p++)
            key[p] = c->lut[(size_t)p * G + cell];
        if (seen.emplace(key, (int)c->tuple_cell.size()).second) {
            c->tuple_cell.push_back(cell);
            for (int w = 0; w < c->TW; w++) {
                uint32_t v = 0;
                for (int b = 0; b < 4; b++) {
                    int p = 4 * w + b;
                    if (p < c->P)
                        v |= (uint32_t)key[p] << (8 * b);
                }
                c->tuples.push_back(v);
            }
        }
    }
    c->U = (int)c->tuple_cell.size();
}

uint16_t bb_query(int P, int K, int p, int lo, int hi)
{
    const int n = hi - lo + 1;
    if (n > 15)
        return 0x1FFF;
    if (lo < 0 || hi >= K || n < 1)
        return 0x1FFF;
    const int lv = n >= 8 ? 3 : (n >= 4 ? 2 : (n >= 2 ? 1 : 0));
    const int KS = tdoa_bb::bb_ks(P, K), PKp = tdoa_bb::bb_pk(P, K), RW = tdoa_bb::bb_row(K);
    int o1;
    if (lv == 0)
        o1 = p * KS + lo;
    else if (P <= 8)
        o1 = lv * PKp + p * K + lo;
    else
        o1 = PKp + (lv - 1) * 4 * RW + (p & 3) * RW + lo;
    if (o1 < 0 || o1 >= 0x1FFF)
        return 0x1FFF;
    return (uint16_t)(o1 | ((n - (1 << lv)) << 13));
}

void build_bb_tiles(tdoa_tables *c, std::vector<int> &all_lo, std::vector<int> &all_hi)
{
    constexpr int TILE = 8, CAP = 64;
    const int P = c->P, TW = c->TW, U = c->U;
    const int tx = (c->W + TILE - 1) / TILE, ty = (c->H + TILE - 1) / TILE;
    std::vector<std::vector<int>> members((size_t)tx * ty);
    for (int u = 0; u < U; u++) {
        const int cell = c->tuple_cell[u];
        const int x = cell % c->W, y = cell / c->W;
        members[(size_t)(y / TILE) * tx + x / TILE].push_back(u);
    }
    std::vector<int32_t> tile;
    std::vector<uint16_t> rng, qry;
    std::vector<uint32_t> tup;
    std::vector<int32_t> uidx;
    all_lo.assign(P, 255);
    all_hi.assign(P, -1);
    for (const auto &m : members)
        for (size_t c0 = 0; c0 < m.size(); c0 += CAP) {
            const size_t n = std::min(m.size() - c0, (size_t)CAP);
            tile.push_back((int32_t)uidx.size());
            tile.push_back((int32_t)n);
            std::vector<int> lo(P, 255), hi(P, 0);
            for (size_t i = 0; i < n; i++) {
                const int u = m[c0 + i];
                uidx.push_back(u);
                for (int w = 0; w < TW; w++)
                    tup.push_back(c->tuples[(size_t)u * TW + w]);
                for (int p = 0; p < P; p++) {
                    const int l = (c->tuples[(size_t)u * TW + p / 4] >> (8 * (p & 3))) & 0xFF;
                    lo[p] = std::min(lo[p], l);
                    hi[p] = std::max(hi[p], l);
                }
            }
            for (int p = 0; p < P; p++) {
                rng.push_back((uint16_t)(lo[p] | (hi[p] << 8)));
                qry.push_back(bb_query(P, c->K, p, lo[p], hi[p]));
                all_lo[p] = std::min(all_lo[p], lo[p]);
                all_hi[p] = std::max(all_hi[p], hi[p]);
            }
        }
    c->bb_NT = (int)tile.size() / 2;
    c->bb_wide = 0;
    for (const uint16_t q : qry)
        c->bb_wide |= (q & 0x1FFF) == 0x1FFF;
    auto put = [&](const void *src, size_t bytes) {
        const size_t at = c->bb_img.size();
        c->bb_img.resize(at + ((bytes + 15) & ~(size_t)15), 0);
        memcpy(c->bb_img.data() + at, src, bytes);
        return at;
    };
    c->bb_img.clear();
    c->bb_at[tdoa_tables::BB_TILE] = put(tile.data(), tile.size() * 4);
    c->bb_at[tdoa_tables::BB_RNG] = put(rng.data(), rng.size() * 2);
    c->bb_at[tdoa_tables::BB_TUPLES] = put(tup.data(), tup.size() * 4);
    c->bb_at[tdoa_tables::BB_UIDX] = put(uidx.data(), uidx.size() * 4);
    c->bb_at[tdoa_tables::BB_Q] = put(qry.data(), qry.size() * 2);
}

void build_compact(tdoa_tables *c, std::vector<int> &lo, const std::vector<int> &hi)
{
    tdoa_kparams &kp = c->kp;
    int off = 0;
    bool ok = c->P <= TDOA_MAX_PAIRS;
    c->wc_chunks.clear();
    const int KS = tdoa_bb::bb_ks(c->P, c->K);
    for (int p = 0; ok && p < c->P; p++) {
        if (c->P > 8 && hi[p] >= lo[p])
            lo[p] &= ~3;
        const int w = hi[p] - lo[p] + 1;
        ok = w > 0 && off < 65536;
        if (!ok)
            break;
        kp.wc_lo[p] = (uint8_t)lo[p];
        kp.wc_w[p] = (uint8_t)w;
        kp.wc_off[p] = (uint16_t)off;
        for (int j = 0; j < w; j += 4)
            c->wc_chunks.push_back((uint32_t)(p * KS + lo[p] + j) | ((uint32_t)std::min(4, w - j) << 16));
        off += (w + 3) & ~3;
    }
    c->wc_ok = ok;
    if (ok) {
        kp.wc_CK = off;
        kp.wc_nch = (int32_t)c->wc_chunks.size();
    }
}

#if TDOA_AB
void build_fused_grid(tdoa_tables *c)
{
    const tdoa_kparams &kp = c->kp;
    const int P = c->P, NT = c->bb_NT;
    const uint16_t *rng = (const uint16_t *)(c->bb_img.data() + c->bb_at[tdoa_tables::BB_RNG]);
    const uint32_t *bt = (const uint32_t *)(c->bb_img.data() + c->bb_at[tdoa_tables::BB_TUPLES]);
    c->fg.assign((size_t)NT * 32, 0);
    c->fg_tup_at = c->fg.size() * 2;
    bool fok = c->wc_ok && kp.wc_CK <= 2048 && NT <= 256 && P <= 32;
    for (int t = 0; fok && t < NT; t++)
        for (int p = 0; p < P; p++) {
            const int lo = rng[(size_t)t * P + p] & 0xFF, hi = rng[(size_t)t * P + p] >> 8;
            const int n = hi - lo + 1;
            if (n < 1 || n > 15 || lo < kp.wc_lo[p] || hi >= kp.wc_lo[p] + kp.wc_w[p]) {
                fok = false;
                break;
            }
            const int lv = n >= 8 ? 3 : (n >= 4 ? 2 : (n >= 2 ? 1 : 0));
            const int e = kp.wc_off[p] + lo - kp.wc_lo[p];
            c->fg[(size_t)t * 32 + p] = (uint16_t)(e | (lv << 11) | ((n - (1 << lv)) << 13));
        }
    c->fg_ok = fok;
    if (!fok)
        return;
    c->fg.resize((size_t)NT * 32 + (size_t)c->U * 32, 0);
    uint16_t *tup = c->fg.data() + (size_t)NT * 32;
    for (int u = 0; u < c->U; u++)
        for (int p = 0; p < P; p++) {
            const int lag = (bt[(size_t)u * c->TW + p / 4] >> (8 * (p & 3))) & 0xFF;
            tup[(size_t)u * 32 + p] = (uint16_t)(kp.wc_off[p] + lag - kp.wc_lo[p]);
        }
}
#endif

int build_window(const tdoa_config *cfg, tdoa_tables *c)
{
    const int N = c->N;
    c->win.resize(N);
    if (cfg->window_q15) {
        for (int i = 0; i < N; i++) {
            if (cfg->window_q15[i] < 0 || cfg->window_q15[i] > 32767)
                return tdoa_fail(TDOA_ERR_INVALID, "window_q15[%d] outside [0,32767]", i);
            c->win[i] = cfg->window_q15[i];
        }
        return TDOA_OK;
    }
    if (N < 1024 && 1024 % N == 0) {
        std::vector<int32_t> w1k(1024);
        const int rc = tdoa_dpss_q15(1024, 2.0, w1k.data());
        for (int i = 0; !rc && i < N; i++)
            c->win[i] = w1k[(size_t)i * (1024 / N)];
        return rc;
    }
    return tdoa_dpss_q15(N, 2.0, c->win.data());
}

void build_twiddles(tdoa_tables *c)
{
    const int N = c->N;
    std::vector<float> &tw = c->tw;
    c->tw2_at = 2 * (size_t)N;
    c->r16_at = 2 * (size_t)N + 2 * ((size_t)N + 1);
    tw.assign(c->r16_at + 2 * 3 * 256, 0.0f);
    for (int k = 0; k < N; k++) {
        const double a = -2.0 * M_PI * k / N;
        tw[2 * k] = (float)std::cos(a);
        tw[2 * k + 1] = (float)std::sin(a);
    }
    for (int k = 0; k <= N; k++) {
        const double a = -2.0 * M_PI * k / (2.0 * N);
        tw[2 * N + 2 * k] = (float)std::cos(a);
        tw[2 * N + 2 * k + 1] = (float)std::sin(a);
    }
    float *t = tw.data() + c->r16_at;
    const int R1 = N >= 256 ? N / 256 : 1;
    const int mul[3] = {R1, 1, 16};
    for (int s = 0; s < 3; s++)
        for (int r = 0; r < 16; r++)
            for (int k = 0; k < 16; k++) {
                const long e = ((long)mul[s] * r * k) % N;
                const double a = -2.0 * M_PI * (double)e / N;
                t[2 * (256 * s + 16 * r + k)] = (float)std::cos(a);
                t[2 * (256 * s + 16 * r + k) + 1] = (float)std::sin(a);
            }
}

void build_kparams(tdoa_tables *c)
{
    const int M = c->M, N = c->N, S = c->S;
    tdoa_kparams &kp = c->kp;
    std::memset(&kp, 0, sizeof kp);
    kp.M = M;
    kp.N = N;
    kp.log2N = ilog2(N);
    kp.P = c->P;
    kp.K = c->K;
    kp.S = S;
    kp.G = c->G;
    kp.U = c->U;
    kp.grid_W = c->W;
    kp.half_w = c->cfg.grid_half_w;
    kp.half_h = c->cfg.grid_half_h;
    kp.grid_scale = c->cfg.grid_scale;
    kp.sbase = (S % 2 == 0) ? -S : -S - 1;
    kp.T = (S - kp.sbase + 1 + TDOA_LT - 1) / TDOA_LT;
    kp.NSEG = (N / 2) / TDOA_SEGW;
    const int need_left = -kp.sbase / 2;
    const int need_right = kp.sbase / 2 + TDOA_LT2 * (kp.T - 1) + TDOA_LT2 + 2;
    kp.PADW = ((std::max(need_left, need_right) + 3) / 4) * 4;
    kp.RS = N / 2 + 2 * kp.PADW;
    kp.TW = c->TW;
    int p = 0;
    for (int i = 0; i < M; i++)
        for (int j = i + 1; j < M; j++, p++) {
            kp.pair_i[p] = (uint8_t)i;
            kp.pair_j[p] = (uint8_t)j;
        }
    kp.fs = (float)c->cfg.sample_rate_hz;
    kp.c = c->cfg.speed_of_sound;
    kp.height = c->cfg.height_offset;
    kp.bb_NT = c->bb_NT;
    kp.bb_wide = c->bb_wide;
}

}

int tdoa_build_tables(const tdoa_config *cfg, tdoa_tables *c)
{
    const int M = cfg->num_mics, N = cfg->frame_len;
    if (M < 2 || M > TDOA_MAX_MICS)
        return tdoa_fail(TDOA_ERR_INVALID, "num_mics %d outside [2,%d]", M, TDOA_MAX_MICS);
    if (N < 256 || N > 4096 || (N & (N - 1)))
        return tdoa_fail(TDOA_ERR_INVALID, "frame_len %d must be a power of two in [256,4096]", N);
    if (cfg->sample_rate_hz <= 0 || !(cfg->speed_of_sound > 0))
        return tdoa_fail(TDOA_ERR_INVALID, "sample_rate_hz / speed_of_sound must be positive");
    const int S = cfg->max_shift > 0 ? cfg->max_shift
                                     : (int)((int64_t)cfg->sample_rate_hz * 32 / 34300);
    if (S < 1 || S > 63)
        return tdoa_fail(TDOA_ERR_INVALID, "max_shift %d outside [1,63]", S);
    if (cfg->engine != TDOA_ENGINE_DIRECT && cfg->engine != TDOA_ENGINE_GCC_PHAT)
        return tdoa_fail(TDOA_ERR_INVALID, "unknown engine %d", cfg->engine);
    if (cfg->grid_half_w < 0 || cfg->grid_half_h < 0 || cfg->grid_half_w > 1000 ||
        cfg->grid_half_h > 1000 || !(cfg->grid_scale > 0) || !(cfg->height_offset > 0))
        return tdoa_fail(TDOA_ERR_INVALID, "bad grid geometry");
    if (M != 3 && !cfg->mic_xy)
        return tdoa_fail(TDOA_ERR_INVALID, "mic_xy is required unless num_mics == 3");

    c->cfg = *cfg;
    c->cfg.mic_xy = nullptr;
    c->cfg.window_q15 = nullptr;
    c->cfg.max_shift = S;
    c->M = M;
    c->N = N;
    c->P = M * (M - 1) / 2;
    c->S = S;
    c->K = 2 * S + 1;
    c->W = 2 * cfg->grid_half_w + 1;
    c->H = 2 * cfg->grid_half_h + 1;
    c->G = c->W * c->H;
    c->TW = (c->P + 3) / 4;

    c->mic.resize(2 * M);
    if (cfg->mic_xy)
        std::memcpy(c->mic.data(), cfg->mic_xy, sizeof(float) * 2 * M);
    else
        reference_triangle(c->mic.data());
    if (const int rc = build_window(cfg, c))
        return rc;
    c->prior.resize(c->K);
    for (int d = 0; d < c->K; d++) {
        const float arg = (float)(-(d * d)) / 36.f;
        c->prior[d] = (float)std::exp((double)arg);
    }
    build_lut(c);
    std::vector<int> lo, hi;
    build_bb_tiles(c, lo, hi);
    build_kparams(c);
    build_compact(c, lo, hi);
    build_twiddles(c);
#if TDOA_AB
    build_fused_grid(c);
#endif
    return TDOA_OK;
}
```

audio-triangulation_amd/csrc/tdoa_tables.h:

```cpp
#pragma once

#include <stddef.h>
#include <stdint.h>

#include <vector>

#include "../../include/tdoa.h"
#include "tdoa_shared.h"

struct tdoa_tables {
    tdoa_config cfg;
    int M, N, P, K, S, G, W, H, U, TW;
    std::vector<float> mic;
    std::vector<int32_t> win;
    std::vector<float> prior;
    std::vector<uint8_t> lut;
    std::vector<uint32_t> tuples;
    std::vector<int32_t> tuple_cell;
    std::vector<float> tw;
    size_t tw2_at, r16_at;
    enum { BB_TILE, BB_RNG, BB_TUPLES, BB_UIDX, BB_Q, BB_SECTIONS };
    std::vector<uint8_t> bb_img;
    size_t bb_at[BB_SECTIONS];
    int bb_NT = 0;
    int bb_wide = 0;
    bool wc_ok = false;
    std::vector<uint32_t> wc_chunks;
#if TDOA_AB
    bool fg_ok = false;
    std::vector<uint16_t> fg;
    size_t fg_tup_at = 0;
#endif
    tdoa_kparams kp;
};

int tdoa_build_tables(const tdoa_config *cfg, tdoa_tables *t);
```

Measured before the change: 152.1 million.

## Make grouped-tuple grid scoring the default path in the 1024-point GCC-PHAT kernel

Replaces the linear tuple scan in the fused GCC-PHAT kernel's grid stage with a grouped layout. Tuples sharing the first two lags and having consecutive third lags are packed into one slot, so each lane scores a fixed 18 slots. Pair partial sums are computed early on half the waves to overlap with the FFT, and third-lag scores are pre-maxed into running-max tables. Exact tie-breaking falls back to a rescan loop. The table image is now built once at table-build time, and the old scan path remains only as an env-selected A/B option. This reduces per-frame grid-scoring work and LDS traffic, but adds tie-handling complexity and fails when the group count exceeds the slot capacity.

```diff
diff --git a/audio-triangulation_amd/csrc/tdoa_capi.cpp b/audio-triangulation_amd/csrc/tdoa_capi.cpp
--- a/audio-triangulation_amd/csrc/tdoa_capi.cpp
+++ b/audio-triangulation_amd/csrc/tdoa_capi.cpp
@@ -107,9 +107,11 @@
     const tdoa_tables &t = c->t;
     if (c->tw.upload(t.tw.data(), vbytes(t.tw)) != hipSuccess)
         return tdoa_fail(TDOA_ERR_NOMEM, "uploading twiddle tables failed");
-    std::vector<uint8_t> img;
-    tdoa_phat1024_image(t.M, t.N, t.K, t.U, t.tw.data(), t.win.data(), t.prior.data(), t.tuples.data(),
-                        t.tuple_cell.data(), img);
+    std::vector<uint8_t> img = t.p1k_img;
+#if TDOA_AB
+    if (!img.empty())
+        img.insert(img.end(), t.p1k_scan_img.begin(), t.p1k_scan_img.end());
+#endif
     if (!img.empty() && c->p1k_img.upload(img.data(), img.size()) != hipSuccess)
         return tdoa_fail(TDOA_ERR_NOMEM, "uploading the GCC_PHAT table image failed");
 #if TDOA_AB
diff --git a/audio-triangulation_amd/csrc/tdoa_internal.h b/audio-triangulation_amd/csrc/tdoa_internal.h
--- a/audio-triangulation_amd/csrc/tdoa_internal.h
+++ b/audio-triangulation_amd/csrc/tdoa_internal.h
@@ -129,9 +129,6 @@
                          const int16_t *frames, int64_t B, float phat_eps,
                          void *spec_scratch, size_t spec_bytes, void *stream);
 bool tdoa_gcc_phat_needs_split(int M, int N);
-void tdoa_phat1024_image(int M, int N, int K, int U, const float *tw, const int32_t *win,
-                         const float *prior, const uint32_t *tuples, const int32_t *tuple_cell,
-                         std::vector<uint8_t> &img);
 void tdoa_p1k_w64_image(int M, int N, int K, int U, const int32_t *win, const float *prior,
                         const uint32_t *tuples, std::vector<uint8_t> &img);
 bool tdoa_gcc_phat_fused_grid(const tdoa_kparams &kp);
diff --git a/audio-triangulation_amd/csrc/tdoa_p1k_layout.h b/audio-triangulation_amd/csrc/tdoa_p1k_layout.h
--- /dev/null
+++ b/audio-triangulation_amd/csrc/tdoa_p1k_layout.h
@@ -0,0 +1,42 @@
+#pragma once
+
+#include <stdint.h>
+
+#include <vector>
+
+#if defined(__HIP__) || defined(__HIPCC__)
+#define TDOA_P1K_HD __host__ __device__
+#else
+#define TDOA_P1K_HD
+#endif
+
+namespace tdoa_p1k {
+
+constexpr int ROW = 264;
+constexpr int TILE = 32 * ROW;
+constexpr int KPAD = 128;
+constexpr int WAVE_LDS = 2 * TILE;
+constexpr int NW = 8;
+constexpr int IMG_FIXED = 32 * 32 * 8 + 16 * 32 * 8 + 512 * 8 + 128 * 4;
+constexpr int IMG_MAX = 4 * NW * 64 * 16;
+
+constexpr int NS = 18;
+constexpr int GRP_HDR = 16;
+constexpr int GRP_BYTES = GRP_HDR + NS * 64 * 4 + NS * 64 * 3 * 2;
+constexpr uint32_t GRP_PAD_WORD = (127u << 3) | (127u << 13) | (127u << 23);
+constexpr int LDS_MAX = 160 * 1024;
+static_assert(IMG_FIXED + GRP_BYTES <= IMG_MAX, "the grouped image exceeds the staging");
+static_assert(NW * WAVE_LDS + IMG_FIXED + GRP_BYTES + 64 <= LDS_MAX, "the grouped image exceeds the LDS");
+static_assert(5 * KPAD * 8 <= WAVE_LDS, "grid score tables exceed the wave's tiles");
+
+TDOA_P1K_HD constexpr int slot(int x) { return x == 16 ? 24 : (x == 24 ? 16 : x); }
+
+}
+
+void tdoa_phat1024_image(int M, int N, int K, int U, const float *tw, const int32_t *win,
+                         const float *prior, const uint32_t *tuples, const int32_t *tuple_cell,
+                         std::vector<uint8_t> &img);
+#if TDOA_AB
+void tdoa_phat1024_scan_image(int M, int N, int K, int U, const float *tw, const int32_t *win,
+                              const float *prior, const uint32_t *tuples, std::vector<uint8_t> &img);
+#endif
diff --git a/audio-triangulation_amd/csrc/tdoa_phat1024.hip b/audio-triangulation_amd/csrc/tdoa_phat1024.hip
--- a/audio-triangulation_amd/csrc/tdoa_phat1024.hip
+++ b/audio-triangulation_amd/csrc/tdoa_phat1024.hip
@@ -1,28 +1,29 @@
 #include <hip/hip_runtime.h>
 #include <stdint.h>
 
-#include <algorithm>
 #include <climits>
 #include <cstdio>
 #include <cstdlib>
-#include <map>
-#include <type_traits>
-#include <vector>
+#include <cstring>
 
 #include "tdoa_cplx.h"
 #include "tdoa_internal.h"
-
+#include "tdoa_p1k_layout.h"
+
+#ifndef TDOA_AB
+#define TDOA_AB 0
+#endif
 
 namespace {
 
-constexpr int P1K_ROW = 264;
-constexpr int P1K_TILE = 32 * P1K_ROW;
-constexpr int P1K_KPAD = 128;
-constexpr int P1K_WAVE_LDS = 2 * P1K_TILE;
-[[maybe_unused]] constexpr int P1K_GB = 8;
-constexpr int P1K_IMG_FIXED = 32 * 32 * 8 + 16 * 32 * 8 + 512 * 8 + 128 * 4;
-
-__host__ __device__ constexpr int slot(int x) { return x == 16 ? 24 : (x == 24 ? 16 : x); }
+using tdoa_p1k::slot;
+constexpr int P1K_ROW = tdoa_p1k::ROW;
+constexpr int P1K_TILE = tdoa_p1k::TILE;
+constexpr int P1K_KPAD = tdoa_p1k::KPAD;
+constexpr int P1K_WAVE_LDS = tdoa_p1k::WAVE_LDS;
+constexpr int P1K_IMG_FIXED = tdoa_p1k::IMG_FIXED;
+constexpr int P1K_NS = tdoa_p1k::NS;
+constexpr int P1K_IMG_GRP = P1K_IMG_FIXED + tdoa_p1k::GRP_BYTES;
 
 __device__ __forceinline__ int lane_res(int l)
 {
@@ -118,11 +119,8 @@
     return *reinterpret_cast<const f2 *>(base + off);
 #endif
 }
-#ifndef P1K_GROUPS
-#define P1K_GROUPS 0
-#endif
-#ifndef P1K_CELL_LDS
-#define P1K_CELL_LDS 0
+#ifndef P1K_ORDER
+#define P1K_ORDER 2
 #endif
 #ifndef P1K_BALANCE
 #define P1K_BALANCE 1
@@ -387,11 +385,9 @@
     swap_upper_exec<false>(v, Ye);
 }
 
-}
-
-__global__ void __launch_bounds__(512, 2) k_p1k_lean(tdoa_kparams kp, tdoa_kout out,
-                                                     const int16_t *__restrict__ frames, int64_t B,
-                                                     float e2)
+template <bool SCAN>
+__device__ __forceinline__ void p1k_lean_body(const tdoa_kparams &kp, const tdoa_kout &out,
+                                              const int16_t *__restrict__ frames, int64_t B, float e2)
 {
     constexpr int N = 1024, P = 3, NW = 8, NF = 2 * NW, NT = NW * 64;
     extern __shared__ __attribute__((aligned(16))) char smem[];
@@ -451,9 +447,9 @@
 
     const int K = kp.K, S = kp.S;
     const bool do_grid = out.cell || out.xy || out.max_Lf;
-#if !P1K_GROUPS
-    const int Upad = (kp.U + P1K_GB * 64 - 1) / (P1K_GB * 64) * (P1K_GB * 64);
-#endif
+    [[maybe_unused]] const int Upad = (kp.U + 511) / 512 * 512;
+    const int img_at = SCAN ? P1K_IMG_GRP : 0;
+    const int img_bytes = SCAN ? kp.p1k_img_bytes - P1K_IMG_GRP : P1K_IMG_GRP;
 
     auto fetch = [&](uint32_t(&w)[16], int64_t fr, int m) {
         const uint32_t *row = reinterpret_cast<const uint32_t *>(
@@ -464,9 +460,9 @@
     };
     uint32_t w0[16], w1[16];
     {
-        const uint4 *src = (const uint4 *)kp.p1k_img;
+        const uint4 *src = (const uint4 *)(static_cast<const char *>(kp.p1k_img) + img_at);
         uint4 *dst = (uint4 *)twm;
-        const int n16 = do_grid ? kp.p1k_img_bytes / 16 : P1K_IMG_FIXED / 16;
+        const int n16 = do_grid ? img_bytes / 16 : P1K_IMG_FIXED / 16;
         constexpr int SR = 4;
         uint4 img[SR];
 #pragma unroll
@@ -577,6 +573,59 @@
         finish_pair(1, y0, y31);
         LEAN_MARK();
         balance();
+        const char *ws = wtiles;
+        const char *ms = wtiles + 2 * P1K_KPAD * 8;
+        const uint32_t *gw = tups + 4 + lane64;
+        auto score_slots = [&](int (&ck)[4], bool (&ok)[4], int &comp, int pad) {
+            const int ft = fresh_tid();
+            const int gres = lane_res_sel(ft & 31);
+            const int gla = 2 * gres, glb = 2 * gres - 64;
+            ck[0] = glb + S, ck[1] = glb + 1 + S, ck[2] = gla + S, ck[3] = gla + 1 + S;
+            ok[0] = glb >= -S, ok[1] = glb + 1 >= -S, ok[2] = gla <= S, ok[3] = gla + 1 <= S;
+            comp = (ft >> 5) & 1;
+            return (ft & 31) == pad;
+        };
+        auto write_w01 = [&]() {
+            float *wsc = (float *)wtiles;
+            int ck[4], comp;
+            bool ok[4];
+#pragma unroll
+            for (int p = 0; p < 2; p++) {
+                const bool pad = score_slots(ck, ok, comp, p);
+#pragma unroll
+                for (int c = 0; c < 4; c++)
+                    if (ok[c])
+                        wsc[(p * P1K_KPAD + ck[c]) * 2 + comp] = wv[p][c];
+                if (pad)
+                    wsc[(p * P1K_KPAD + P1K_KPAD - 1) * 2 + comp] = -INFINITY;
+            }
+        };
+        f2 gpart[P1K_NS];
+        uint32_t gmo[P1K_NS];
+        auto partial_grid = [&]() {
+            wave_lds_sync();
+            write_w01();
+            wave_lds_sync();
+            uint32_t w[P1K_NS];
+#pragma unroll
+            for (int s = 0; s < P1K_NS; s++)
+                w[s] = lds_rd_u32(gw + 64 * s);
+#pragma unroll
+            for (int s = 0; s < P1K_NS; s++) {
+                gpart[s] = lds_f2_plain(ws, (int)(w[s] & 0x3FFu)) +
+                           lds_f2_plain(ws, P1K_KPAD * 8 + (int)((w[s] >> 10) & 0x3FFu));
+                gmo[s] = w[s] >> 20;
+            }
+#pragma unroll
+            for (int s = 0; s < P1K_NS; s++)
+                pin(gpart[s]);
+            LEAN_MARK();
+            balance();
+        };
+        const int swave = __builtin_amdgcn_readfirstlane(wave);
+        const bool pg_early = !SCAN && do_grid && (P1K_ORDER == 2 ? !(swave & 4) : P1K_ORDER == 1);
+        if (pg_early)
+            partial_grid();
         {
             f2 v[32];
             lean_pretwiddle<false>(L, U1, U1, v);
@@ -604,269 +653,215 @@
 #endif
             return;
         }
-        wave_lds_sync();
-#if P1K_CELL_LDS && !P1K_GROUPS
-        float *wsc = (float *)(((uintptr_t)wtiles + 1023) & ~(uintptr_t)1023);
-#else
-        float *wsc = (float *)wtiles;
-#endif
-        const int gres = lane_res_sel(fresh_tid() & 31);
-        const int gla = 2 * gres, glb = 2 * gres - 64;
-        const int ck[4] = {glb + S, glb + 1 + S, gla + S, gla + 1 + S};
-        const bool ok[4] = {glb >= -S, glb + 1 >= -S, gla <= S, gla + 1 <= S};
-#pragma unroll
-        for (int p = 0; p < P; p++)
-#pragma unroll
-            for (int c = 0; c < 4; c++)
-                if (ok[c])
-                    wsc[(p * P1K_KPAD + ck[c]) * 2 + hw] = wv[p][c];
-        {
-            const int ft = fresh_tid();
-            if ((ft & 31) < 3)
-                wsc[((ft & 31) * P1K_KPAD + P1K_KPAD - 1) * 2 + ((ft >> 5) & 1)] = -INFINITY;
+        float gv[2] = {-INFINITY, -INFINITY};
+        int wcell[2];
+        if constexpr (!SCAN) {
+            if (!pg_early)
+                partial_grid();
+            wave_lds_sync();
+            {
+                float *msc = (float *)(wtiles + 2 * P1K_KPAD * 8);
+                int ck[4], comp;
+                bool ok[4];
+                const bool pad = score_slots(ck, ok, comp, 2);
+#pragma unroll
+                for (int c = 0; c < 4; c++)
+                    if (ok[c])
+                        msc[ck[c] * 2 + comp] = wv[2][c];
+                if (pad)
+                    msc[(P1K_KPAD - 1) * 2 + comp] = -INFINITY;
+                wave_lds_sync();
+                typedef float f4 __attribute__((ext_vector_type(4)));
+                const int l64 = fresh_tid() & 63;
+                const f4 lo = *reinterpret_cast<const f4 *>(msc + 4 * l64);
+                f4 hi = *reinterpret_cast<const f4 *>(msc + 4 * (l64 < 63 ? l64 + 1 : 63));
+                if (l64 == 63)
+                    hi = f4{-INFINITY, -INFINITY, -INFINITY, -INFINITY};
+                f4 m2, m3;
+                m2.x = fmaxf(lo.x, lo.z), m2.y = fmaxf(lo.y, lo.w);
+                m2.z = fmaxf(lo.z, hi.x), m2.w = fmaxf(lo.w, hi.y);
+                m3.x = fmaxf(m2.x, hi.x), m3.y = fmaxf(m2.y, hi.y);
+                m3.z = fmaxf(m2.z, hi.z), m3.w = fmaxf(m2.w, hi.w);
+                *reinterpret_cast<f4 *>(msc + 2 * P1K_KPAD + 4 * l64) = m2;
+                *reinterpret_cast<f4 *>(msc + 4 * P1K_KPAD + 4 * l64) = m3;
+            }
+            wave_lds_sync();
+            LEAN_MARK();
+            int gs[2] = {0, 0};
+            float gp[2] = {0.0f, 0.0f};
+            uint64_t seen[2] = {0, 0}, tied[2] = {0, 0};
+            {
+                f2 Lg[P1K_NS];
+#pragma unroll
+                for (int s = 0; s < P1K_NS; s++)
+                    Lg[s] = gpart[s] + lds_f2_plain(ms, (int)gmo[s]);
+#pragma unroll
+                for (int s = 0; s < P1K_NS; s++) {
+                    gv[0] = fmaxf(gv[0], Lg[s].x);
+                    gv[1] = fmaxf(gv[1], Lg[s].y);
+                }
+#pragma unroll
+                for (int s = P1K_NS - 1; s >= 0; s--) {
+                    const float v[2] = {Lg[s].x, Lg[s].y}, pt[2] = {gpart[s].x, gpart[s].y};
+#pragma unroll
+                    for (int j = 0; j < 2; j++) {
+                        const bool eq = v[j] == gv[j];
+                        const uint64_t mk = __ballot(eq);
+                        tied[j] |= mk & seen[j];
+                        seen[j] |= mk;
+                        gs[j] = eq ? s : gs[j];
+                        gp[j] = eq ? pt[j] : gp[j];
+                    }
+                }
+            }
+            LEAN_MARK();
+            const uint16_t *gcl = reinterpret_cast<const uint16_t *>(tups + 4 + P1K_NS * 64);
+            int cand[2];
+#pragma unroll
+            for (int j = 0; j < 2; j++) {
+                const int sl = gs[j] * 64 + lane64;
+                const uint32_t w = tups[4 + sl];
+                const int nm1 = (int)(w >> 30), mo = (int)((w >> 20) & 0x3FFu);
+                int mc = INT_MAX;
+#pragma unroll
+                for (int i = 0; i < 3; i++) {
+                    const f2 m1 = lds_f2_plain(ms, mo + 8 * i);
+                    const float Li = gp[j] + (j ? m1.y : m1.x);
+                    const int ci = gcl[3 * sl + i];
+                    if (i <= nm1 && Li == gv[j])
+                        mc = imin(mc, ci);
+                }
+                cand[j] = gv[j] > -INFINITY ? mc : INT_MAX;
+            }
+            bool tie[2];
+#pragma unroll
+            for (int j = 0; j < 2; j++) {
+                int gk = fkey(gv[j]);
+                wave_argmax_key(gk, cand[j]);
+                const float V = fkey_value(gk);
+                tie[j] = (tied[j] & __ballot(gv[j] == V && V > -INFINITY)) != 0;
+                gv[j] = V;
+            }
+            if (tie[0] || tie[1]) {
+                wave_lds_sync();
+                write_w01();
+                wave_lds_sync();
+                int mc[2] = {INT_MAX, INT_MAX};
+#pragma unroll 1
+                for (int s = 0; s < P1K_NS; s++) {
+                    const int sl = s * 64 + lane64;
+                    const uint32_t w = tups[4 + sl];
+                    const f2 part = lds_f2_plain(ws, (int)(w & 0x3FFu)) +
+                                    lds_f2_plain(ws, P1K_KPAD * 8 + (int)((w >> 10) & 0x3FFu));
+                    const int nm1 = (int)(w >> 30), mo = (int)((w >> 20) & 0x3FFu);
+#pragma unroll
+                    for (int i = 0; i < 3; i++) {
+                        const f2 Li = part + lds_f2_plain(ms, mo + 8 * i);
+                        const int ci = gcl[3 * sl + i];
+                        if (i <= nm1 && Li.x == gv[0])
+                            mc[0] = imin(mc[0], ci);
+                        if (i <= nm1 && Li.y == gv[1])
+                            mc[1] = imin(mc[1], ci);
+                    }
+                }
+#pragma unroll
+                for (int j = 0; j < 2; j++)
+                    if (tie[j])
+                        cand[j] = wave_reduce<false>(mc[j]);
+            }
+#pragma unroll
+            for (int j = 0; j < 2; j++)
+                wcell[j] = cand[j] == INT_MAX ? (int)tups[3] : cand[j];
+            LEAN_MARK();
         }
-        wave_lds_sync();
-        LEAN_MARK();
-#if P1K_GROUPS
-        const int *ghdr = reinterpret_cast<const int *>(static_cast<const char *>(kp.p1k_img) + P1K_IMG_FIXED);
-        const int gn3 = ghdr[0], gn2 = ghdr[1], gn1 = ghdr[2], gcell0 = ghdr[3];
-        const uint32_t *gw = tups + 4;
-        const uint16_t *gcl = reinterpret_cast<const uint16_t *>(gw + gn3 + gn2 + gn1);
-        const int gcb2 = 3 * gn3, gcb1 = gcb2 + 2 * gn2, gend = gn3 + gn2 + gn1;
-        float gv[2] = {-INFINITY, -INFINITY};
-        int gs[2] = {0, 0}, gsl[2] = {0, 0};
-        const char *ws = (const char *)wsc;
-        constexpr int R1 = P1K_KPAD * 8, R2 = 2 * P1K_KPAD * 8;
-        auto gat = [&](auto nm, uint32_t w, f2 &a, f2 &b, f2 (&c)[decltype(nm)::value]) {
-            a = lds_rd(reinterpret_cast<const f2 *>(ws + (w & 0x3FFu)));
-            b = lds_rd(reinterpret_cast<const f2 *>(ws + R1 + ((w >> 10) & 0x3FFu)));
-#pragma unroll
-            for (int j = 0; j < decltype(nm)::value; j++)
-                c[j] = lds_rd(reinterpret_cast<const f2 *>(ws + R2 + (w >> 20) + 8 * j));
-        };
-        auto bucket = [&](auto nm, int s0, int s1) {
-            constexpr int NM = decltype(nm)::value;
-            if (s0 >= s1)
-                return;
-            const int last = s1 - 64;
-            const int nu = (s1 - s0) / 128;
-            auto words = [&](uint32_t (&w)[2], int u) {
-                w[0] = lds_rd_u32(gw + imin(s0 + 128 * u, last) + lane64);
-                w[1] = lds_rd_u32(gw + imin(s0 + 128 * u + 64, last) + lane64);
+#if TDOA_AB
+        else {
+            wave_lds_sync();
+            float *wsc = (float *)wtiles;
+            const int gres = lane_res_sel(fresh_tid() & 31);
+            const int gla = 2 * gres, glb = 2 * gres - 64;
+            const int ck[4] = {glb + S, glb + 1 + S, gla + S, gla + 1 + S};
+            const bool ok[4] = {glb >= -S, glb + 1 >= -S, gla <= S, gla + 1 <= S};
+#pragma unroll
+            for (int p = 0; p < P; p++)
+#pragma unroll
+                for (int c = 0; c < 4; c++)
+                    if (ok[c])
+                        wsc[(p * P1K_KPAD + ck[c]) * 2 + hw] = wv[p][c];
+            {
+                const int ft = fresh_tid();
+                if ((ft & 31) < 3)
+                    wsc[((ft & 31) * P1K_KPAD + P1K_KPAD - 1) * 2 + ((ft >> 5) & 1)] = -INFINITY;
+            }
+            wave_lds_sync();
+            LEAN_MARK();
+            int gu[2] = {INT_MAX, INT_MAX};
+            auto gather = [&](const uint32_t (&qq)[4], f2 (&g)[4][3]) {
+#pragma unroll
+                for (int i = 0; i < 4; i++) {
+                    g[i][0] = lds_f2_plain(ws, (int)(qq[i] & 0x3FFu));
+                    g[i][1] = lds_f2_plain(ws, P1K_KPAD * 8 + (int)((qq[i] >> 10) & 0x3FFu));
+                    g[i][2] = lds_f2_plain(ws, 2 * P1K_KPAD * 8 + (int)(qq[i] >> 20));
+                }
             };
-            auto gather = [&](const uint32_t (&w)[2], f2 (&a)[2], f2 (&b)[2], f2 (&c)[2][NM]) {
-                gat(nm, w[0], a[0], b[0], c[0]);
-                gat(nm, w[1], a[1], b[1], c[1]);
-            };
-            auto consume = [&](const f2 (&a)[2], const f2 (&b)[2], const f2 (&c)[2][NM], int u) {
-#pragma unroll
-                for (int r = 0; r < 2; r++) {
-                    const f2 part = a[r] + b[r];
-                    f2 L[NM];
-#pragma unroll
-                    for (int j = 0; j < NM; j++)
-                        L[j] = part + c[r][j];
-                    float m[2] = {L[0].x, L[0].y};
-#pragma unroll
-                    for (int j = 1; j < NM; j++) {
-                        m[0] = fmaxf(m[0], L[j].x);
-                        m[1] = fmaxf(m[1], L[j].y);
+            uint32_t q[4];
+            f2 g[4][3];
+#pragma unroll
+            for (int i = 0; i < 4; i++)
+                q[i] = tups[64 * i + lane64];
+            gather(q, g);
+            auto consume = [&](const f2 (&gg)[4][3], int ub) {
+#pragma unroll
+                for (int i = 0; i < 4; i++) {
+                    const f2 Lg = (gg[i][0] + gg[i][1]) + gg[i][2];
+                    const int u = ub + 64 * i + lane64;
+                    if (Lg.x > gv[0]) {
+                        gv[0] = Lg.x;
+                        gu[0] = u;
                     }
-                    const int sl = s0 + 128 * u + 64 * r + lane64;
-#pragma unroll
-                    for (int f = 0; f < 2; f++) {
-                        const bool gt = m[f] > gv[f];
-                        gsl[f] = m[f] >= gv[f] ? sl : gsl[f];
-                        gs[f] = gt ? sl : gs[f];
-                        gv[f] = gt ? m[f] : gv[f];
+                    if (Lg.y > gv[1]) {
+                        gv[1] = Lg.y;
+                        gu[1] = u;
                     }
                 }
             };
-            f2 a0[2], b0[2], c0[2][NM], a1[2], b1[2], c1[2][NM];
-            uint32_t w2[2], w3[2];
-            words(w2, 0);
-            gather(w2, a0, b0, c0);
-            words(w3, 1);
-            words(w2, 2);
-            gather(w3, a1, b1, c1);
-            int u = 0;
-            for (; u + 3 < nu; u += 2) {
-                consume(a0, b0, c0, u);
-                words(w3, u + 3);
-                gather(w2, a0, b0, c0);
-                __builtin_amdgcn_sched_barrier(0);
-                consume(a1, b1, c1, u + 1);
-                words(w2, u + 4);
-                gather(w3, a1, b1, c1);
-                __builtin_amdgcn_sched_barrier(0);
-            }
-            consume(a0, b0, c0, u);
-            if (u + 2 < nu)
-                gather(w2, a0, b0, c0);
-            if (u + 1 < nu)
-                consume(a1, b1, c1, u + 1);
-            if (u + 2 < nu)
-                consume(a0, b0, c0, u + 2);
-        };
-        bucket(std::integral_constant<int, 3>{}, 0, gn3);
-        bucket(std::integral_constant<int, 2>{}, gn3, gn3 + gn2);
-        bucket(std::integral_constant<int, 1>{}, gn3 + gn2, gend);
-        LEAN_MARK();
-        auto group_cell = [&](int sl, int f, float v) {
-            const int nm = sl < gn3 ? 3 : (sl < gn3 + gn2 ? 2 : 1);
-            const int cb = sl < gn3 ? 3 * sl : (sl < gn3 + gn2 ? gcb2 + 2 * (sl - gn3) : gcb1 + (sl - gn3 - gn2));
-            const uint32_t w = gw[sl];
-            const f2 part = lds_f2_plain(ws, (int)(w & 0x3FFu)) + lds_f2_plain(ws, R1 + (int)((w >> 10) & 0x3FFu));
-            int mc = INT_MAX;
-#pragma unroll
-            for (int j = 0; j < 3; j++) {
-                if (j < nm) {
-                    const f2 Lg = part + lds_f2_plain(ws, R2 + (int)(w >> 20) + 8 * j);
-                    if ((f ? Lg.y : Lg.x) == v)
-                        mc = imin(mc, (int)gcl[cb + j]);
-                }
-            }
-            return mc;
-        };
-        int cand[2];
-        {
-            uint32_t bw[2];
-            int bnm[2], bc[2][3];
-#pragma unroll
-            for (int f = 0; f < 2; f++) {
-                const int sl = gs[f];
-                bnm[f] = sl < gn3 ? 3 : (sl < gn3 + gn2 ? 2 : 1);
-                const int cb = sl < gn3 ? 3 * sl : (sl < gn3 + gn2 ? gcb2 + 2 * (sl - gn3) : gcb1 + (sl - gn3 - gn2));
-                bw[f] = gw[sl];
-#pragma unroll
-                for (int j = 0; j < 3; j++)
-                    bc[f][j] = gcl[cb + imin(j, bnm[f] - 1)];
-            }
-#pragma unroll
-            for (int f = 0; f < 2; f++) {
-                const uint32_t w = bw[f];
-                const f2 part = lds_f2_plain(ws, (int)(w & 0x3FFu)) + lds_f2_plain(ws, R1 + (int)((w >> 10) & 0x3FFu));
-                int mc = INT_MAX;
-#pragma unroll
-                for (int j = 0; j < 3; j++) {
-                    const f2 Lg = part + lds_f2_plain(ws, R2 + (int)(w >> 20) + 8 * j);
-                    if (j < bnm[f] && (f ? Lg.y : Lg.x) == gv[f])
-                        mc = imin(mc, bc[f][j]);
-                }
-                cand[f] = gv[f] > -INFINITY ? mc : INT_MAX;
-            }
-        }
-        int wcell[2];
-#pragma unroll
-        for (int j = 0; j < 2; j++) {
-            int ci = cand[j];
-            int gk = fkey(gv[j]);
-            wave_argmax_key(gk, ci);
-            const float V = fkey_value(gk);
-            if (__ballot(gsl[j] != gs[j] && gv[j] == V && V > -INFINITY)) {
-                int mc = INT_MAX;
-                for (int sl = lane64; sl < gend; sl += 64)
-                    mc = imin(mc, group_cell(sl, j, V));
-                ci = wave_reduce<false>(mc);
-            }
-            wcell[j] = ci == INT_MAX ? gcell0 : ci;
-            gv[j] = V;
-        }
-        LEAN_MARK();
-#else
-        float gv[2] = {-INFINITY, -INFINITY};
-        int gu[2] = {INT_MAX, INT_MAX};
-        const char *ws = (const char *)wsc;
-#if P1K_CELL_LDS
-        const uint32_t wsb = (uint32_t)(uintptr_t)(const __attribute__((address_space(3))) char *)ws;
-#endif
-        auto gather = [&](const uint32_t (&qq)[4], f2 (&g)[4][3]) {
-#pragma unroll
-            for (int i = 0; i < 4; i++) {
-#if P1K_CELL_LDS
-                g[i][0] = lds_at((qq[i] & 0x3F8u) | wsb);
-                g[i][1] = lds_at((((qq[i] >> 7) & 0x3F8u) | wsb) + P1K_KPAD * 8);
-                g[i][2] = lds_at((((qq[i] >> 14) & 0x3F8u) | wsb) + 2 * P1K_KPAD * 8);
-#else
-                g[i][0] = lds_f2_plain(ws, (int)(qq[i] & 0x3FFu));
-                g[i][1] = lds_f2_plain(ws, P1K_KPAD * 8 + (int)((qq[i] >> 10) & 0x3FFu));
-                g[i][2] = lds_f2_plain(ws, 2 * P1K_KPAD * 8 + (int)(qq[i] >> 20));
-#endif
-            }
-        };
-        uint32_t q[4];
-        f2 g[4][3];
-#pragma unroll
-        for (int i = 0; i < 4; i++)
-            q[i] = tups[64 * i + lane64];
-        gather(q, g);
-        auto consume = [&](const f2 (&gg)[4][3], int ub) {
-#pragma unroll
-            for (int i = 0; i < 4; i++) {
-                const f2 Lg = (gg[i][0] + gg[i][1]) + gg[i][2];
-                const int u = ub + 64 * i + lane64;
-                if (Lg.x > gv[0]) {
-                    gv[0] = Lg.x;
-                    gu[0] = u;
-                }
-                if (Lg.y > gv[1]) {
-                    gv[1] = Lg.y;
-                    gu[1] = u;
-                }
-            }
-        };
-        for (int u0 = 0; u0 < Upad; u0 += 512) {
-            uint32_t qn[4];
-#pragma unroll
-            for (int i = 0; i < 4; i++)
-                qn[i] = tups[u0 + 256 + 64 * i + lane64];
-            f2 gn[4][3];
-            gather(qn, gn);
-            consume(g, u0);
-            const int un = u0 + 512 < Upad ? u0 + 512 : u0 + 256;
-#pragma unroll
-            for (int i = 0; i < 4; i++)
-                q[i] = tups[un + 64 * i + lane64];
-            gather(q, g);
-            consume(gn, u0 + 256);
-        }
-        LEAN_MARK();
-        int mycell[2], myu[2];
-#if P1K_CELL_LDS
-        const int *rowcell = reinterpret_cast<const int *>(tups + Upad);
-#pragma unroll
-        for (int j = 0; j < 2; j++) {
-            myu[j] = gu[j];
-            const int uc = (gu[j] < 0 || gu[j] >= kp.U) ? 0 : gu[j];
-            const uint32_t tw = tups[uc];
-            mycell[j] = rowcell[uc >> 5] + (int)((tw >> 24) | ((tw & 7u) << 8));
-        }
-#else
-#pragma unroll
-        for (int j = 0; j < 2; j++) {
-            myu[j] = gu[j];
-            mycell[j] = kp.tuple_cell[(gu[j] < 0 || gu[j] >= kp.U) ? 0 : gu[j]];
-        }
-#endif
-        int gk[2];
-#pragma unroll
-        for (int j = 0; j < 2; j++) {
-            gk[j] = fkey(gv[j]);
-            wave_argmax_key(gk[j], gu[j]);
-            gv[j] = fkey_value(gk[j]);
-        }
-        LEAN_MARK();
-        int wcell[2];
-#if P1K_CELL_LDS
-        const int tuple_cell0 = rowcell[0];
-#else
-        const int tuple_cell0 = kp.tuple_cell[0];
-#endif
-#pragma unroll
-        for (int j = 0; j < 2; j++) {
-            const int fu = gu[j];
-            const uint64_t wm = __ballot(myu[j] == fu && fu >= 0 && fu < kp.U);
-            wcell[j] = wm ? __builtin_amdgcn_readlane(mycell[j], __builtin_ctzll(wm)) : tuple_cell0;
+            for (int u0 = 0; u0 < Upad; u0 += 512) {
+                uint32_t qn[4];
+#pragma unroll
+                for (int i = 0; i < 4; i++)
+                    qn[i] = tups[u0 + 256 + 64 * i + lane64];
+                f2 gn[4][3];
+                gather(qn, gn);
+                consume(g, u0);
+                const int un = u0 + 512 < Upad ? u0 + 512 : u0 + 256;
+#pragma unroll
+                for (int i = 0; i < 4; i++)
+                    q[i] = tups[un + 64 * i + lane64];
+                gather(q, g);
+                consume(gn, u0 + 256);
+            }
+            LEAN_MARK();
+            int mycell[2], myu[2];
+#pragma unroll
+            for (int j = 0; j < 2; j++) {
+                myu[j] = gu[j];
+                mycell[j] = kp.tuple_cell[(gu[j] < 0 || gu[j] >= kp.U) ? 0 : gu[j]];
+            }
+            int gk[2];
+#pragma unroll
+            for (int j = 0; j < 2; j++) {
+                gk[j] = fkey(gv[j]);
+                wave_argmax_key(gk[j], gu[j]);
+                gv[j] = fkey_value(gk[j]);
+            }
+            LEAN_MARK();
+            const int tuple_cell0 = kp.tuple_cell[0];
+#pragma unroll
+            for (int j = 0; j < 2; j++) {
+                const int fu = gu[j];
+                const uint64_t wm = __ballot(myu[j] == fu && fu >= 0 && fu < kp.U);
+                wcell[j] = wm ? __builtin_amdgcn_readlane(mycell[j], __builtin_ctzll(wm)) : tuple_cell0;
+            }
         }
 #endif
         if (lane64 == 63) {
@@ -902,6 +897,23 @@
 #undef LEAN_MARK
 }
 
+}
+
+__global__ void __launch_bounds__(512, 2) k_p1k_lean(tdoa_kparams kp, tdoa_kout out,
+                                                     const int16_t *__restrict__ frames, int64_t B,
+                                                     float e2)
+{
+    p1k_lean_body<false>(kp, out, frames, B, e2);
+}
+#if TDOA_AB
+__global__ void __launch_bounds__(512, 2) k_p1k_lean_scan(tdoa_kparams kp, tdoa_kout out,
+                                                          const int16_t *__restrict__ frames, int64_t B,
+                                                          float e2)
+{
+    p1k_lean_body<true>(kp, out, frames, B, e2);
+}
+#endif
+
 #ifdef TDOA_DIAG
 extern "C" int tdoa_diag_fetch_p1k(unsigned long long *host, int n)
 {
@@ -915,124 +927,21 @@
 #endif
 
 namespace {
-constexpr int P1K_NW = 8;
+constexpr int P1K_NW = tdoa_p1k::NW;
 
 constexpr size_t p1k_lds(int img_bytes) { return (size_t)P1K_NW * P1K_WAVE_LDS + (size_t)img_bytes; }
-}
-
-void tdoa_phat1024_image(int M, int N, int K, int U, const float *tw, const int32_t *win,
-                         const float *prior, const uint32_t *tuples, const int32_t *tuple_cell,
-                         std::vector<uint8_t> &img)
-{
-    img.clear();
-    if (M != 3 || N != 1024 || K > P1K_KPAD - 1)
-        return;
-#if P1K_GROUPS
-    struct Grp {
-        int l0, l1, l2, n, u0;
-        int cell[3];
-    };
-    std::map<std::pair<int, int>, std::vector<std::pair<int, int>>> by;
-    for (int u = 0; u < U; u++)
-        by[{(int)(tuples[u] & 0xFFu), (int)((tuples[u] >> 8) & 0xFFu)}].push_back({(int)((tuples[u] >> 16) & 0xFFu), u});
-    std::vector<Grp> bk[4];
-    for (auto &kv : by) {
-        auto &v = kv.second;
-        std::sort(v.begin(), v.end());
-        for (size_t i = 0; i < v.size();) {
-            Grp g{kv.first.first, kv.first.second, v[i].first, 0, INT_MAX, {0, 0, 0}};
-            while (i < v.size() && g.n < 3 && v[i].first == g.l2 + g.n) {
-                if (tuple_cell[v[i].second] < 0 || tuple_cell[v[i].second] >= 0xFFFF)
-                    return;
-                g.cell[g.n++] = tuple_cell[v[i].second];
-                g.u0 = std::min(g.u0, v[i].second);
-                i++;
-            }
-            bk[g.n].push_back(g);
-        }
-    }
-    int nslot[4];
-    for (int n = 1; n <= 3; n++) {
-        std::sort(bk[n].begin(), bk[n].end(), [](const Grp &x, const Grp &y) { return x.u0 < y.u0; });
-        nslot[n] = ((int)bk[n].size() + 127) / 128 * 128;
-    }
-    const int ncell = 3 * nslot[3] + 2 * nslot[2] + nslot[1];
-    const size_t bytes = (size_t)P1K_IMG_FIXED + 16 + 4 * (size_t)(nslot[3] + nslot[2] + nslot[1]) + 2 * (size_t)ncell;
-    img.resize((bytes + 15) / 16 * 16);
-#else
-    const int Upad = (U + P1K_GB * 64 - 1) / (P1K_GB * 64) * (P1K_GB * 64);
-#if P1K_CELL_LDS
-    img.resize((size_t)P1K_IMG_FIXED + (size_t)Upad * 4 + (size_t)(Upad / 32) * 4);
-#else
-    (void)tuple_cell;
-    img.resize((size_t)P1K_IMG_FIXED + (size_t)Upad * 4);
-#endif
-#endif
-    float *f = (float *)img.data();
-    const float *tw2 = tw + 2 * N;
-    for (int k = 0; k < 32; k++)
-        for (int r = 0; r < 32; r++) {
-            const int i = (k * r) & (N - 1);
-            f[2 * (32 * k + slot(r))] = tw[2 * i];
-            f[2 * (32 * k + slot(r)) + 1] = tw[2 * i + 1];
-        }
-    f += 2 * 1024;
-    for (int k = 0; k < 16; k++)
-        for (int r = 0; r < 32; r++) {
-            const int b = r + 32 * k;
-            f[2 * (32 * k + slot(r))] = tw2[2 * b];
-            f[2 * (32 * k + slot(r)) + 1] = tw2[2 * b + 1];
-        }
-    f += 2 * 512;
-    for (int e = 0; e < 512; e++) {
-        const int d = (e & ~31) + slot(e & 31);
-        f[2 * d] = (float)win[2 * e] * (1.0f / 128.0f);
-        f[2 * d + 1] = (float)win[2 * e + 1] * (1.0f / 128.0f);
-    }
-    f += 2 * 512;
-    for (int k = 0; k < 128; k++)
-        f[k] = k < K ? prior[k] : 0.0f;
-    uint32_t *t = (uint32_t *)(f + 128);
-#if P1K_GROUPS
-    int32_t *hdr = (int32_t *)t;
-    hdr[0] = nslot[3];
-    hdr[1] = nslot[2];
-    hdr[2] = nslot[1];
-    hdr[3] = U > 0 ? tuple_cell[0] : 0;
-    t += 4;
-    uint16_t *cl = (uint16_t *)(t + nslot[3] + nslot[2] + nslot[1]);
-    for (int n = 3; n >= 1; n--) {
-        for (int e = 0; e < nslot[n]; e++) {
-            const bool real = e < (int)bk[n].size();
-            const Grp g = real ? bk[n][e] : Grp{127, 127, 128 - n, n, 0, {0xFFFF, 0xFFFF, 0xFFFF}};
-            *t++ = ((uint32_t)g.l0 << 3) | ((uint32_t)g.l1 << 13) | ((uint32_t)g.l2 << 23);
-            for (int j = 0; j < n; j++)
-                *cl++ = (uint16_t)g.cell[j];
-        }
-    }
-#else
-#if P1K_CELL_LDS
-    int32_t *rowcell = (int32_t *)(t + Upad);
-    for (int r = 0; r < Upad / 32; r++) {
-        const int e0 = 32 * r, e1 = std::min(U, e0 + 32) - 1;
-        rowcell[r] = e0 >= U ? 0 : tuple_cell[e0];
-        if (e0 < U && tuple_cell[e1] - tuple_cell[e0] >= 2048) {
-            img.clear();
-            return;
-        }
-    }
-    for (int e = 0; e < Upad; e++) {
-        const uint32_t wd = e < U ? tuples[e] : 0x007F7F7Fu;
-        const uint32_t dc = e < U ? (uint32_t)(tuple_cell[e] - rowcell[e >> 5]) : 0u;
-        t[e] = ((wd & 0x7Fu) << 3) | (((wd >> 8) & 0x7Fu) << 10) | (((wd >> 16) & 0x7Fu) << 17) |
-               ((dc & 0xFFu) << 24) | (dc >> 8);
-    }
-#else
-    for (int e = 0; e < Upad; e++) {
-        const uint32_t wd = e < U ? tuples[e] : 0x007F7F7Fu;
-        t[e] = ((wd & 0xFFu) << 3) | (((wd >> 8) & 0xFFu) << 13) | (((wd >> 16) & 0xFFu) << 23);
-    }
-#endif
+
+#if TDOA_AB
+bool p1k_use_scan(const tdoa_kparams &kp)
+{
+    static const bool want = [] {
+        const char *e = getenv("TDOA_P1K_GRID");
+        return e && !strcmp(e, "scan");
+    }();
+    const int bytes = kp.p1k_img_bytes - P1K_IMG_GRP;
+    return want && bytes > P1K_IMG_FIXED && bytes <= tdoa_p1k::IMG_MAX &&
+           p1k_lds(bytes) + 64 <= (size_t)tdoa_p1k::LDS_MAX;
+}
 #endif
 }
 
@@ -1040,8 +949,7 @@
 {
     if (kp.M != 3 || kp.N != 1024 || kp.S > 63 || kp.TW != 1 || !kp.p1k_img)
         return false;
-    static_assert(3 * P1K_KPAD * 8 <= P1K_WAVE_LDS, "grid scores exceed the wave's tiles");
-    return kp.p1k_img_bytes <= 4 * P1K_NW * 64 * 16 && p1k_lds(kp.p1k_img_bytes) + 64 <= 160 * 1024;
+    return kp.p1k_img_bytes >= P1K_IMG_GRP;
 }
 
 int tdoa_launch_phat1024(const tdoa_kparams &kp, const tdoa_kout &out, const int16_t *frames,
@@ -1056,8 +964,14 @@
     const int64_t grid = (B + NF - 1) / NF;
     if (grid > 0x7FFFFFFF)
         return tdoa_set_error(-1, "k_p1k_lean: batch too large for one launch");
-    hipLaunchKernelGGL(k_p1k_lean, dim3((unsigned)grid), dim3(P1K_NW * 64), p1k_lds(kp.p1k_img_bytes), (hipStream_t)stream,
-                       kp, out, frames, B, e2);
+#if TDOA_AB
+    if (p1k_use_scan(kp))
+        hipLaunchKernelGGL(k_p1k_lean_scan, dim3((unsigned)grid), dim3(P1K_NW * 64),
+                           p1k_lds(kp.p1k_img_bytes - P1K_IMG_GRP), (hipStream_t)stream, kp, out, frames, B, e2);
+    else
+#endif
+        hipLaunchKernelGGL(k_p1k_lean, dim3((unsigned)grid), dim3(P1K_NW * 64), p1k_lds(P1K_IMG_GRP),
+                           (hipStream_t)stream, kp, out, frames, B, e2);
     const hipError_t e = hipGetLastError();
     if (e != hipSuccess) {
         char buf[256];
diff --git a/audio-triangulation_amd/csrc/tdoa_tables.cpp b/audio-triangulation_amd/csrc/tdoa_tables.cpp
--- a/audio-triangulation_amd/csrc/tdoa_tables.cpp
+++ b/audio-triangulation_amd/csrc/tdoa_tables.cpp
@@ -2,8 +2,10 @@
 #include "tdoa_tables.h"
 
 #include "tdoa_bb_layout.h"
+#include "tdoa_p1k_layout.h"
 
 #include <algorithm>
+#include <climits>
 #include <cmath>
 #include <cstdarg>
 #include <cstdio>
@@ -500,7 +502,109 @@
     kp.bb_wide = c->bb_wide;
 }
 
-}
+uint8_t *p1k_fixed_image(int N, int K, const float *tw, const int32_t *win, const float *prior, uint8_t *img)
+{
+    using tdoa_p1k::slot;
+    float *f = (float *)img;
+    const float *tw2 = tw + 2 * N;
+    for (int k = 0; k < 32; k++)
+        for (int r = 0; r < 32; r++) {
+            const int i = (k * r) & (N - 1);
+            f[2 * (32 * k + slot(r))] = tw[2 * i];
+            f[2 * (32 * k + slot(r)) + 1] = tw[2 * i + 1];
+        }
+    f += 2 * 1024;
+    for (int k = 0; k < 16; k++)
+        for (int r = 0; r < 32; r++) {
+            const int b = r + 32 * k;
+            f[2 * (32 * k + slot(r))] = tw2[2 * b];
+            f[2 * (32 * k + slot(r)) + 1] = tw2[2 * b + 1];
+        }
+    f += 2 * 512;
+    for (int e = 0; e < 512; e++) {
+        const int d = (e & ~31) + slot(e & 31);
+        f[2 * d] = (float)win[2 * e] * (1.0f / 128.0f);
+        f[2 * d + 1] = (float)win[2 * e + 1] * (1.0f / 128.0f);
+    }
+    f += 2 * 512;
+    for (int k = 0; k < 128; k++)
+        f[k] = k < K ? prior[k] : 0.0f;
+    return (uint8_t *)(f + 128);
+}
+
+}
+
+void tdoa_phat1024_image(int M, int N, int K, int U, const float *tw, const int32_t *win,
+                         const float *prior, const uint32_t *tuples, const int32_t *tuple_cell,
+                         std::vector<uint8_t> &img)
+{
+    using namespace tdoa_p1k;
+    img.clear();
+    if (M != 3 || N != 1024 || K > KPAD - 1 || U < 1)
+        return;
+    struct Grp {
+        int l0, l1, l2, n, u0;
+        int cell[3];
+    };
+    std::map<std::pair<int, int>, std::vector<std::pair<int, int>>> by;
+    for (int u = 0; u < U; u++)
+        by[{(int)(tuples[u] & 0xFFu), (int)((tuples[u] >> 8) & 0xFFu)}].push_back({(int)((tuples[u] >> 16) & 0xFFu), u});
+    std::vector<Grp> grp;
+    for (auto &kv : by) {
+        auto &v = kv.second;
+        std::sort(v.begin(), v.end());
+        for (size_t i = 0; i < v.size();) {
+            Grp g{kv.first.first, kv.first.second, v[i].first, 0, INT_MAX, {0xFFFF, 0xFFFF, 0xFFFF}};
+            if (g.l0 >= K || g.l1 >= K)
+                return;
+            while (i < v.size() && g.n < 3 && v[i].first == g.l2 + g.n) {
+                const int u = v[i].second;
+                if (tuple_cell[u] < 0 || tuple_cell[u] >= 0xFFFF || v[i].first >= K)
+                    return;
+                g.cell[g.n++] = tuple_cell[u];
+                g.u0 = std::min(g.u0, u);
+                i++;
+            }
+            grp.push_back(g);
+        }
+    }
+    if (grp.size() > (size_t)NS * 64)
+        return;
+    std::sort(grp.begin(), grp.end(), [](const Grp &x, const Grp &y) { return x.u0 < y.u0; });
+    img.assign((size_t)IMG_FIXED + GRP_BYTES, 0);
+    int32_t *hdr = (int32_t *)p1k_fixed_image(N, K, tw, win, prior, img.data());
+    hdr[0] = (int32_t)grp.size();
+    hdr[1] = NS * 64;
+    hdr[3] = tuple_cell[0];
+    uint32_t *t = (uint32_t *)(hdr + 4);
+    uint16_t *cl = (uint16_t *)(t + NS * 64);
+    for (int e = 0; e < NS * 64; e++) {
+        const bool real = e < (int)grp.size();
+        t[e] = real ? ((uint32_t)grp[e].l0 << 3) | ((uint32_t)grp[e].l1 << 13) |
+                          ((uint32_t)((grp[e].n - 1) * KPAD + grp[e].l2) << 23)
+                    : GRP_PAD_WORD;
+        for (int j = 0; j < 3; j++)
+            cl[3 * e + j] = real ? (uint16_t)grp[e].cell[j] : 0xFFFF;
+    }
+}
+
+#if TDOA_AB
+void tdoa_phat1024_scan_image(int M, int N, int K, int U, const float *tw, const int32_t *win,
+                              const float *prior, const uint32_t *tuples, std::vector<uint8_t> &img)
+{
+    using namespace tdoa_p1k;
+    img.clear();
+    if (M != 3 || N != 1024 || K > KPAD - 1)
+        return;
+    const int Upad = (U + 511) / 512 * 512;
+    img.assign((size_t)IMG_FIXED + (size_t)Upad * 4, 0);
+    uint32_t *t = (uint32_t *)p1k_fixed_image(N, K, tw, win, prior, img.data());
+    for (int e = 0; e < Upad; e++) {
+        const uint32_t wd = e < U ? tuples[e] : 0x007F7F7Fu;
+        t[e] = ((wd & 0xFFu) << 3) | (((wd >> 8) & 0xFFu) << 13) | (((wd >> 16) & 0xFFu) << 23);
+    }
+}
+#endif
 
 int tdoa_build_tables(const tdoa_config *cfg, tdoa_tables *c)
 {
@@ -555,7 +659,11 @@
     build_kparams(c);
     build_compact(c, lo, hi);
     build_twiddles(c);
+    tdoa_phat1024_image(M, N, c->K, c->U, c->tw.data(), c->win.data(), c->prior.data(), c->tuples.data(),
+                        c->tuple_cell.data(), c->p1k_img);
 #if TDOA_AB
+    tdoa_phat1024_scan_image(M, N, c->K, c->U, c->tw.data(), c->win.data(), c->prior.data(), c->tuples.data(),
+                             c->p1k_scan_img);
     build_fused_grid(c);
 #endif
     return TDOA_OK;
diff --git a/audio-triangulation_amd/csrc/tdoa_tables.h b/audio-triangulation_amd/csrc/tdoa_tables.h
--- a/audio-triangulation_amd/csrc/tdoa_tables.h
+++ b/audio-triangulation_amd/csrc/tdoa_tables.h
@@ -26,7 +26,9 @@
     int bb_wide = 0;
     bool wc_ok = false;
     std::vector<uint32_t> wc_chunks;
+    std::vector<uint8_t> p1k_img;
 #if TDOA_AB
+    std::vector<uint8_t> p1k_scan_img;
     bool fg_ok = false;
     std::vector<uint16_t> fg;
     size_t fg_tup_at = 0;
```

New measurement: 152.3 million, median of 2. Within noise of the previous version (+0.1%).
